# TrevorS/voxtral-mini-realtime-rs

Hardware: AMD Instinct MI355X
Metric: decode_tok_per_s (higher is better)
Workload: dtype f32

## Files before the change

voxtral-mini-realtime-rs_amd/csrc/vox_api.cpp:

```cpp
#include "vox_page_pool.h"
#include "vox_dev_base.h"
#include "vox_snapshot.h"
#include "vox_kv_bf16.h"

#include <algorithm>
#include <array>
#include <cassert>
#include <cmath>
#include <cstdio>
#include <cstdlib>
#include <cstring>
#include <deque>
#include <map>
#include <string>
#include <thread>
#include <vector>

using namespace vox;
using namespace vox_host;

namespace vox_host {
void binding_release(EngBinding& b) {
    for (void* p : {(void*)b.tab, (void*)b.part_val, (void*)b.part_idx}) if (p) (void)hipFree(p);
    if (b.err_word) (void)hipHostFree(b.err_word);
// ... 374 lines not shown
        if (f.w2 == PF::W2_F32) return q4_linear_dev(cx, L->w2.w, nullptr, ffn, F, M, x, D, EPI_RESID, x, D);
        if (f.w2 == PF::W2_PLANES_ROWS) HIPCHK(launch_xf_rows(ffn, F, M, F, cx->xf_scratch, s));
        return planes_from_xf(L->w2.w, f.kz_w2);
    };
    for (int l = 0; l < c.dec_layers; l++) {
        L = &m->dec[l]; kl = kc->k + (size_t)l * kc->layer_stride; vl = kc->v + (size_t)l * kc->layer_stride;
        VOXCHK(forms[l].f32_rows() ? layer_f32() : layer_xf(forms[l], l ? forms[l - 1].kz_w2 : 0));
    }
    if (!forms.empty() && forms.back().kz_w2) HIPCHK(launch_splitk_finish_resid(cx->kz_scratch, forms.back().kz_w2, M, D, x, D, s));
    return VOX_OK;
}

static bool decode_layer_fuses_attn_wo(const vox_model* m, const DecLayer& L, const AttnParams& ap, const vox_cache* kc) {
    const vox_model_cfg& c = m->cfg; const int D = c.dec_dim;
    return attn_wo_supported(ap, L.wo.w, c.dec_head_dim, kc->max_seq) && L.w13.w.fmt == WFMT_Q4_0 && L.w2.w.fmt == WFMT_Q4_0  && L.wo.w.N == D && D % 4 == 0 && L.w13.w.K == 3072 &&
           q4_gemv_default_R(L.w13.w.N, L.w13.w.K, EPI_SWIGLU) == 2;
}

static int32_t wo_acc_clear(vox_model* m, hipStream_t s) { if (m->d_wo_acc) HIPCHK(hipMemsetAsync(m->d_wo_acc, 0, (size_t)m->cfg.dec_layers * m->cfg.dec_dim * 8, s)); return VOX_OK; }
struct DecRingStep { const float* rope; int mask; };
static int32_t decoder_step_dev(vox_model* m, float* h, vox_cache* kc, const int* pos_ptr, int pos_off, const DecRingStep* ring = nullptr) {
    const vox_model_cfg& c = m->cfg; hipStream_t s = m->ctx->stream;
    const int D = c.dec_dim, H = c.dec_heads, KV = c.dec_kv_heads, hd = c.dec_head_dim, QD = H * hd, KD = KV * hd, F = c.dec_ffn;
    const size_t lf = kc->layer_stride;
    for (int l = 0; l < c.dec_layers; l++) {
        const DecLayer& L = m->dec[l]; float* kl = kc->k + (size_t)l * lf; float* vl = kc->v + (size_t)l * lf;
        GemvParams p{};
        p.w = L.wqkv.w; p.x = h; p.x_stride = D; p.out = m->d_q; p.out_stride = QD; p.gamma = L.attn_norm; p.eps = c.norm_eps;
        p.pos_ptr = pos_ptr; p.pos_off = pos_off; p.rope_cos = m->dec_cos; p.rope_sin = m->dec_sin; p.hd = hd; p.n_q = QD; p.n_k = KD;
        p.kcache = kl; p.vcache = vl; p.cache_head_stride = kc->max_seq * hd;
        if (ring) { p.rope_cos = ring->rope; p.rope_sin = ring->rope + hd / 2; p.rope_mask = ring->mask; }
        {
            HIPCHK(launch_q4_gemv(p, 1, PRO_RMS, ring ? EPI_ROPE_KV_RING : EPI_ROPE_KV, q4_gemv_default_R(p.w.N, p.w.K, EPI_ROPE_KV), s));
            AttnParams ap{}; ap.q = m->d_q; ap.k = kl; ap.v = vl; ap.kv_row_stride = hd; ap.kv_head_stride = kc->max_seq * hd; ap.out = m->d_att;
            ap.n_heads = H; ap.n_kv_heads = KV; ap.offset = pos_off; ap.window = c.dec_window; ap.pos_ptr = pos_ptr; ap.M = 1; ap.spec_rows = kc->max_seq;
            const int R13 = q4_gemv_default_R(L.w13.w.N, L.w13.w.K, EPI_SWIGLU);
            if (!ring && decode_layer_fuses_attn_wo(m, L, ap, kc) && h != m->d_h2) {
                long long* acc = m->d_wo_acc + (size_t)l * D;
                HIPCHK(launch_attn_wo(ap, L.wo.w, acc, kc->max_seq, s));
                GemvParams f{}; f.w = L.w13.w; f.x = h; f.x_stride = D; f.out = m->d_act; f.out_stride = F; f.gamma = L.ffn_norm; f.mul = L.ada_mul; f.eps = c.norm_eps;
                f.xacc = acc; f.x_out = m->d_h2;
                HIPCHK(launch_q4_gemv(f, 1, PRO_RMS_MUL_SUM, EPI_SWIGLU, R13, s));
                GemvParams d{}; d.w = L.w2.w; d.x = m->d_act; d.x_stride = F; d.out = h; d.out_stride = D; d.resid = m->d_h2; d.resid_stride = D;
                d.zero_acc = acc; d.zero_n = D;
                HIPCHK(launch_q4_gemv(d, 1, PRO_NONE, EPI_RESID, q4_gemv_default_R(d.w.N, d.w.K, EPI_RESID), s));
                continue;
            }
            HIPCHK(ring ? launch_attn_decode_ring(ap, hd, kc->max_seq, s) : launch_attn_decode(ap, hd, kc->max_seq, s));
        }
        GemvParams o{}; o.w = L.wo.w; o.x = m->d_att; o.x_stride = QD; o.out = h; o.out_stride = D; o.resid = h; o.resid_stride = D;
        HIPCHK(launch_q4_gemv(o, 1, PRO_NONE, EPI_RESID, q4_gemv_default_R(o.w.N, o.w.K, EPI_RESID), s));
        GemvParams f{}; f.w = L.w13.w; f.x = h; f.x_stride = D; f.out = m->d_act; f.out_stride = F; f.gamma = L.ffn_norm; f.mul = L.ada_mul; f.eps = c.norm_eps;
        HIPCHK(launch_q4_gemv(f, 1, PRO_RMS_MUL, EPI_SWIGLU, q4_gemv_default_R(f.w.N, f.w.K, EPI_SWIGLU), s));
        GemvParams d{}; d.w = L.w2.w; d.x = m->d_act; d.x_stride = F; d.out = h; d.out_stride = D; d.resid = h; d.resid_stride = D;
        HIPCHK(launch_q4_gemv(d, 1, PRO_NONE, EPI_RESID, q4_gemv_default_R(d.w.N, d.w.K, EPI_RESID), s));
    }
    return VOX_OK;
}

static int32_t engine_stream_prepare(vox_model* m) {
    const vox_model_cfg& c = m->cfg; hipStream_t s = m->ctx->stream;
    if (m->eng_ready || !m->eng_ok) return VOX_OK;
    const size_t sb = eng_stream_bytes(c.dec_layers, c.vocab);
    if (!m->eng_stream) {
        hipError_t e = hipMalloc((void**)&m->eng_stream, sb);
        if (e == hipSuccess) e = hipMalloc((void**)&m->eng_state, eng_state_bytes());
        if (e != hipSuccess) {
            (void)hipGetLastError();
            if (m->eng_stream) (void)hipFree(m->eng_stream); if (m->eng_state) (void)hipFree(m->eng_state);
            m->eng_stream = nullptr; m->eng_state = nullptr; m->eng_ok = false; m->eng_on = false; m->engb_ok = false;
            fprintf(stderr, "[voxtral_hip] decode engine: allocating the %.2f GB weight stream failed (%s); the launch-based decode paths are used\n", sb / 1e9, hipGetErrorString(e));
            return VOX_OK;
        }
    }
    HIPCHK(hipMemsetAsync(m->eng_stream, 0, sb, s)); HIPCHK(hipMemsetAsync(m->eng_state, 0, eng_state_bytes(), s));
    for (int l = 0; l < c.dec_layers; l++) {
        const DecLayer& L = m->dec[l];
        HIPCHK(launch_eng_pack(L.wqkv.w, 0, l, c.dec_layers, m->eng_stream, c.vocab, s)); HIPCHK(launch_eng_pack(L.wo.w, 1, l, c.dec_layers, m->eng_stream, c.vocab, s));
        HIPCHK(launch_eng_pack(L.w13.w, 2, l, c.dec_layers, m->eng_stream, c.vocab, s)); HIPCHK(launch_eng_pack(L.w2.w, 3, l, c.dec_layers, m->eng_stream, c.vocab, s));
    }
    HIPCHK(launch_eng_pack(m->tok.w, 4, 0, c.dec_layers, m->eng_stream, c.vocab, s));
    m->eng_ready = true;
    return VOX_OK;
}
static bool engb_prepare(vox_model* m, int n_grp) {
    if (!m->engb_ok || !m->engb_on || n_grp > 4) return false;
    if (engine_stream_prepare(m) != VOX_OK || !m->eng_ready) return false;
    if (engb_prepare_kernels() != hipSuccess) { (void)hipGetLastError(); m->engb_ok = false; return false; }
    if (!m->eng_wob) {
        const vox_model_cfg& c = m->cfg; hipStream_t s = m->ctx->stream;
        hipError_t e = hipMalloc((void**)&m->eng_wob, engb_wo_stream_bytes(c.dec_layers));
        if (e == hipSuccess) e = hipMemsetAsync(m->eng_wob, 0, engb_wo_stream_bytes(c.dec_layers), s);
        for (int l = 0; l < c.dec_layers && e == hipSuccess; l++) e = launch_eng_pack(m->dec[l].wo.w, 5, l, c.dec_layers, m->eng_wob, c.vocab, s);
        if (e != hipSuccess) { (void)hipGetLastError(); if (m->eng_wob) { (void)hipFree(m->eng_wob); m->eng_wob = nullptr; } m->engb_ok = false; return false; }
    }
    for (int gi = 0; gi < n_grp; gi++) {
        if (m->engb_state[gi]) continue;
        hipError_t e = hipMalloc((void**)&m->engb_state[gi], engb_state_bytes());
        if (e == hipSuccess) e = hipMalloc((void**)&m->engb_tab[gi], sizeof(EngLayerTab) * 32);
        if (e == hipSuccess) e = engb_state_init(m->engb_state[gi], m->ctx->stream);
        if (e != hipSuccess) { (void)hipGetLastError(); if (m->engb_state[gi]) { (void)hipFree(m->engb_state[gi]); m->engb_state[gi] = nullptr; } return false; }
    }
    return true;
}
static int32_t engine_strike(vox_model* m) {
    m->eng_strikes++;
    HIPCHK(hipMemsetAsync(m->eng_state, 0, eng_state_bytes(), m->ctx->stream)); m->eng_launches = 0; graphs_destroy(m);
    if (m->eng_strikes >= 3) { m->eng_ok = false; m->eng_on = false; }
    return VOX_OK;
}
static const int ENGINE_MAX_ROWS = 1024;
static void dec_layer_tab(const vox_model* m, float* k, float* v, size_t layer_stride, size_t group_off, EngLayerTab* out) {
    for (size_t l = 0, o = group_off; l < (size_t)m->cfg.dec_layers; l++, o += layer_stride) out[l] = EngLayerTab{m->dec[l].attn_norm, m->dec[l].ffn_norm, m->dec[l].ada_mul, k + o, v + o};
}
static bool engine_serves(const vox_model* m, const vox_cache* kc) { return m->eng_ok && m->eng_on && !m->eng_suspended && kc && kc->max_seq <= ENGINE_MAX_ROWS; }
static hipError_t engine_tab_enqueue(vox_model* m, EngBinding& b, const vox_cache* kc) {
    b.host.resize(m->cfg.dec_layers); dec_layer_tab(m, kc->k, kc->v, kc->layer_stride, 0, b.host.data());
    const hipError_t e = hipMemcpyAsync(b.tab, b.host.data(), sizeof(EngLayerTab) * b.host.size(), hipMemcpyHostToDevice, m->ctx->stream);
    b.cache = e == hipSuccess ? kc : nullptr; b.gen = kc->gen; return e;
}
static hipError_t binding_alloc(const vox_model* m, EngBinding& b, uint64_t* bytes = nullptr) {
    hipError_t e = hipSuccess; auto A = [&](void** q, size_t n) { if (e == hipSuccess && !*q && (e = hipMalloc(q, n)) == hipSuccess && bytes) *bytes += n; };
    A((void**)&b.tab, sizeof(EngLayerTab) * std::max(m->cfg.dec_layers, 32)); A((void**)&b.part_val, 256 * 4); A((void**)&b.part_idx, 256 * 4);
    if (e == hipSuccess && !b.err_word) { e = hipHostMalloc((void**)&b.err_word, 8, hipHostMallocDefault); if (e == hipSuccess) b.err_word[0] = b.err_word[1] = 0u; else b.err_word = nullptr; }
    return e;
}
static bool engine_bind(vox_model* m, EngBinding& b, const vox_cache* kc) {
    if (!engine_serves(m, kc) || engine_stream_prepare(m) != VOX_OK || !m->eng_ready) return false;
    hipError_t e = binding_alloc(m, b);
    if (e == hipSuccess && (b.cache != kc || b.gen != kc->gen)) { e = engine_tab_enqueue(m, b, kc); if (e == hipSuccess) e = hipStreamSynchronize(m->ctx->stream); }
    if (e != hipSuccess) { (void)hipGetLastError(); b.cache = nullptr; }
    return e == hipSuccess;
}
static EngParams engine_params(vox_model* m, const EngBinding& b, const vox_cache* kc, const float* h_in, const int* pos_ptr, int pos_off, float* logits_out) {
    const vox_model_cfg& c = m->cfg;
    EngParams ep{}; ep.stream = m->eng_stream; ep.cu_stride = eng_stream_bytes(c.dec_layers, c.vocab) / 256; ep.layers = b.tab; ep.n_layers = c.dec_layers; ep.h_in = h_in; ep.final_norm = m->dec_norm;
    ep.pos_ptr = pos_ptr; ep.pos_off = pos_off; ep.rope_cos = m->dec_cos; ep.rope_sin = m->dec_sin; ep.max_seq = kc->max_seq; ep.window = c.dec_window; ep.eps = c.norm_eps;
    eng_state_carve(m->eng_state, &ep); ep.part_val = b.part_val; ep.part_idx = b.part_idx; ep.logits_out = logits_out; ep.vocab = c.vocab; ep.tl = nullptr; ep.tl_layer = -1;
    ep.flags = m->eng_flags; ep.pace_ticks = (m->eng_flags & 512) ? 0 : m->eng_pace; ep.ag_delay_ticks = (m->eng_flags & 512) ? m->eng_pace : 0;
    return ep;
}
static int32_t engine_take_serials(vox_model* m, unsigned long long n, hipStream_t s) {
    if (m->eng_launches + n > (1ull << 25)) { HIPCHK(hipMemsetAsync(m->eng_state, 0, eng_state_bytes(), s)); m->eng_launches = 0; }
    m->eng_launches += n; return VOX_OK;
}
static int32_t engine_err_enqueue(vox_model* m, unsigned* dst, hipStream_t s) {
    EngParams ep{}; eng_state_carve(m->eng_state, &ep); HIPCHK(hipMemcpyAsync(dst, ep.err, 8, hipMemcpyDeviceToHost, s)); return VOX_OK;
}
static std::string engine_timeout_text(unsigned e, int strikes) {
    char b[96]; const int n = snprintf(b, sizeof b, "hand-off timeout (code %u, workgroup %u)", e & 0xff, (e >> 8) & 0xff);
    if (strikes > 0) snprintf(b + n, sizeof b - n, ", strike %d of 3", strikes);
    return b;
}
struct EngSuspend { vox_model* m; bool was; explicit EngSuspend(vox_model* m_) : m(m_), was(m_->eng_suspended) { m->eng_suspended = true; } ~EngSuspend() { m->eng_suspended = was; } };

extern "C" int32_t vox_model_set_decode_engine(vox_model* m, int32_t on, int32_t* active) {
    ARGCHK(m, "null argument"); VOXCHK(ctx_bind(m->ctx));
    const bool want = on != 0 && m->eng_ok;
    if (want != m->eng_on) { HIPCHK(hipStreamSynchronize(m->ctx->stream)); graphs_destroy(m); m->eng_on = want; }
    if (active) *active = m->eng_on ? 1 : 0;
    return VOX_OK;
}

extern "C" int32_t vox_model_set_batch_engine(vox_model* m, int32_t on, int32_t* active, uint64_t* launches) {
    ARGCHK(m, "null argument");
    if (on >= 0) m->engb_on = on != 0;
    if (active) *active = m->engb_ok && m->engb_on ? 1 : 0;
    if (launches) *launches = m->engb_launches;
    return VOX_OK;
}

static int32_t lm_head_argmax_dev(vox_model* m, const float* h, float* logits_out) {
    const vox_model_cfg& c = m->cfg;
    ARGCHK(c.dec_dim <= 4096, "lm_head GEMV is instantiated for dec_dim <= 4096 (got %d)", c.dec_dim);
    GemvParams p{}; p.w = m->tok.w; p.x = h; p.x_stride = c.dec_dim; p.out = logits_out; p.out_stride = c.vocab; p.gamma = m->dec_norm; p.eps = c.norm_eps;
    p.part_val = m->d_part_val; p.part_idx = m->d_part_idx;
    if (m->tok.w.fmt == WFMT_Q4_0) m->n_parts = q4_gemv_grid_k(c.vocab, c.dec_dim, m->argmax_R, EPI_ARGMAX);
    HIPCHK(launch_q4_gemv(p, 1, PRO_RMS, EPI_ARGMAX, m->argmax_R, m->ctx->stream));
    return VOX_OK;
}

static int32_t ensure_decode_state(vox_model* m, int S) {
    if (!m->cache || m->cache->max_seq < S) {
        int cap = std::max(S, 256); cap = std::min((cap + 255) / 256 * 256, m->dec_rope_len);
        ARGCHK(S <= cap, "sequence of %d decoder positions exceeds the RoPE table (%d)", S, m->dec_rope_len);
        if (m->cache) { HIPCHK(hipStreamSynchronize(m->ctx->stream)); cache_release(m->cache); m->eng_offline.cache = nullptr; }
        graphs_destroy(m);
        VOXCHK(cache_alloc(m, cap, &m->cache));
    }
    if (!m->d_tokens) { m->tokens_cap = m->dec_rope_len + 2; HIPCHK(hipMalloc((void**)&m->d_tokens, (size_t)m->tokens_cap * 4)); }
    ARGCHK(S + 2 <= m->tokens_cap, "sequence of %d decoder positions exceeds the token buffer", S);
    return VOX_OK;
}

namespace vox_host {
void prefix_release(vox_model* m) {
    PrefixState& p = m->pfx;
    for (float** q : {&p.enc_kv, &p.audio, &p.dec_k, &p.dec_v}) { if (*q) (void)hipFree(*q); *q = nullptr; }
    p.enc_built = p.dec_built = false; p.enc_bytes = p.dec_bytes = 0; p.t_embed.clear();
}
}
static void prefix_bounds(const vox_model* m, int* RC, int* PC) {
    const vox_model_cfg& c = m->cfg; *RC = 0; *PC = 0;
    vox_pad_cfg pc; vox_pad_cfg_voxtral(&pc);
    const long left = (long)pad_left(&pc), R = c.reshape_factor;
    if (left < 200 || R < 1 || c.n_mels != 128 || (c.enc_head_dim != 64 && c.enc_head_dim != 128) || m->enc.empty() || m->dec.empty()) return;
    const long Fc = (left - 200) / 160, rows = Fc >= 3 ? (Fc - 3) / 4 + 1 : 0;
    const long pcn = VOX_PREFIX_TOKENS - 1;
    if (rows / R < pcn || pcn * R + 4 > m->enc_rope_len) return;
    *PC = (int)pcn; *RC = (int)(pcn * R);
}
static bool prefix_active(const vox_model* m) { int rc, pc; prefix_bounds(m, &rc, &pc); return m->pfx.on && rc > 0; }
static hipError_t prefix_tokens_enqueue(int* d_tokens, hipStream_t s) { return hipMemcpyAsync(d_tokens, PREFIX_TOKENS.t, sizeof PREFIX_TOKENS.t, hipMemcpyHostToDevice, s); }
static int32_t prefill_prefix_rows(vox_model* m, const float* audio, int rows) {
    const vox_model_cfg& c = m->cfg;
    if (!m->d_prefix) HIPCHK(hipMalloc((void**)&m->d_prefix, (size_t)VOX_PREFIX_TOKENS * c.dec_dim * 4));
    HIPCHK(launch_embed(m->tok.w, m->d_tokens, rows, audio, c.dec_dim, nullptr, 0, 0, m->d_prefix, m->ctx->stream));
    m->cache->len = 0;
    return decoder_prefill_dev(m, m->d_prefix, rows, m->cache, 0);
}
static int32_t prefix_build(vox_model* m, const float* t_embed) {
    PrefixState& p = m->pfx; const vox_model_cfg& c = m->cfg; vox_ctx* cx = m->ctx; hipStream_t s = cx->stream;
    int RC, PC; prefix_bounds(m, &RC, &PC);
    if (!p.on || RC <= 0) return VOX_OK;
    if (p.enc_built && p.dec_built && p.t_embed.size() == (size_t)c.dec_dim && !std::memcmp(p.t_embed.data(), t_embed, (size_t)c.dec_dim * 4)) return VOX_OK;
    const int QD = c.enc_heads * c.enc_head_dim, hd = c.dec_head_dim, KV = c.dec_kv_heads;
    p.RC = RC; p.PC = PC;
    const size_t rows_bytes = (size_t)PC * hd * 4, n_rows = (size_t)c.dec_layers * KV;
    {
        hipError_t e = hipSuccess;
        auto A = [&](float** q, size_t n) { if (e == hipSuccess && !*q) e = hipMalloc((void**)q, n); };
        A(&p.enc_kv, (size_t)c.enc_layers * RC * 2 * QD * 4); A(&p.audio, (size_t)PC * c.dec_dim * 4); A(&p.dec_k, rows_bytes * n_rows); A(&p.dec_v, rows_bytes * n_rows);
        if (e != hipSuccess) {
            (void)hipGetLastError(); prefix_release(m); p.on = false;
            fprintf(stderr, "[voxtral_hip] prefix state: allocating %.1f MB failed (%s); every call runs the full computation\n",
                    ((double)c.enc_layers * RC * 2 * QD * 4 + 2.0 * rows_bytes * n_rows) / 1e6, hipGetErrorString(e));
            return VOX_OK;
        }
    }
    if (!p.enc_built) {
        const int Tb = 4 * (RC + 4);
        p.enc_bytes = (uint64_t)c.enc_layers * RC * 2 * QD * 4 + (uint64_t)PC * c.dec_dim * 4;
        MelTables t; VOXCHK(ctx_mel_tables(cx, &t));
        DevBuf mel; HIPCHK(mel.alloc((size_t)c.n_mels * Tb * 4));
        HIPCHK(launch_mel(nullptr, 0, (long)Tb * 160, 0, nullptr, t, mel.as<float>(), Tb, 1, s));
        int S4 = 0; p.capture = p.enc_kv; p.capture_rows = RC;
        const int32_t r = encode_dev(m, mel.as<float>(), Tb, &S4);
        p.capture = nullptr; p.capture_rows = 0;
        VOXCHK(r); ARGCHK(S4 >= PC, "internal: prefix build gave %d audio rows", S4);
        HIPCHK(hipMemcpyAsync(p.audio, m->d_audio, (size_t)PC * c.dec_dim * 4, hipMemcpyDeviceToDevice, s));
        HIPCHK(hipStreamSynchronize(s));
        p.enc_built = true;
    }
    VOXCHK(vox_model_set_t_embed(m, t_embed));
    VOXCHK(ensure_decode_state(m, VOX_PREFIX_TOKENS));
    p.dec_bytes = 2 * (uint64_t)rows_bytes * n_rows;
    HIPCHK(prefix_tokens_enqueue(m->d_tokens, s));
    VOXCHK(prefill_prefix_rows(m, p.audio, PC));
    const size_t pitch = (size_t)m->cache->max_seq * hd * 4;
    ARGCHK(m->cache->layer_stride == (size_t)KV * m->cache->max_seq * hd, "internal: cache layout");
    HIPCHK(hipMemcpy2DAsync(p.dec_k, rows_bytes, m->cache->k, pitch, rows_bytes, n_rows, hipMemcpyDeviceToDevice, s));
    HIPCHK(hipMemcpy2DAsync(p.dec_v, rows_bytes, m->cache->v, pitch, rows_bytes, n_rows, hipMemcpyDeviceToDevice, s));
    HIPCHK(hipStreamSynchronize(s));
    p.t_embed.assign(t_embed, t_embed + c.dec_dim); p.dec_built = true;
    return VOX_OK;
}
static int32_t prefix_rows_into(vox_model* m, vox_cache* kc, hipStream_t s) {
    const vox_model_cfg& c = m->cfg; const PrefixState& P = m->pfx;
    const size_t rows_bytes = (size_t)P.PC * c.dec_head_dim * 4, n_rows = (size_t)c.dec_layers * c.dec_kv_heads, pitch = (size_t)kc->max_seq * c.dec_head_dim * 4;
    const size_t plane = (size_t)c.dec_kv_heads * kc->max_seq * c.dec_head_dim, src_layer = (size_t)c.dec_kv_heads * P.PC * c.dec_head_dim;
    if (kc->layer_stride == plane) {
        HIPCHK(hipMemcpy2DAsync(kc->k, pitch, P.dec_k, rows_bytes, rows_bytes, n_rows, hipMemcpyDeviceToDevice, s));
        HIPCHK(hipMemcpy2DAsync(kc->v, pitch, P.dec_v, rows_bytes, rows_bytes, n_rows, hipMemcpyDeviceToDevice, s));
    } else for (int l = 0; l < c.dec_layers; l++) {
        HIPCHK(hipMemcpy2DAsync(kc->k + (size_t)l * kc->layer_stride, pitch, P.dec_k + (size_t)l * src_layer, rows_bytes, rows_bytes, c.dec_kv_heads, hipMemcpyDeviceToDevice, s));
        HIPCHK(hipMemcpy2DAsync(kc->v + (size_t)l * kc->layer_stride, pitch, P.dec_v + (size_t)l * src_layer, rows_bytes, rows_bytes, c.dec_kv_heads, hipMemcpyDeviceToDevice, s));
    }
    kc->len = P.PC; return VOX_OK;
}
static bool prefix_usable(const vox_model* m, int T) {
    const PrefixState& p = m->pfx; const vox_model_cfg& c = m->cfg;
    if (!p.on || !p.enc_built || !p.dec_built || p.RC <= 0 || knob_str("VOX_ATTN_F32")) return false;
    const int S = enc_rows(T);
    return S / c.reshape_factor > VOX_PREFIX_TOKENS && S <= m->enc_rope_len;
}
extern "C" int32_t vox_model_set_prefix_cache(vox_model* m, int32_t on, int32_t* active) {
    ARGCHK(m, "null argument"); VOXCHK(ctx_bind(m->ctx));
    if (on >= 0) {
        m->pfx.on = on != 0;
        if (!m->pfx.on) { HIPCHK(hipStreamSynchronize(m->ctx->stream)); prefix_release(m); }
        else if (m->t_embed_set) { std::vector<float> te = m->t_embed_host; VOXCHK(prefix_build(m, te.data())); }
    }
    if (active) *active = prefix_active(m) ? 1 : 0;
    return VOX_OK;
}
extern "C" int32_t vox_model_prefix_info(const vox_model* m, int32_t out[4]) {
    ARGCHK(m && out, "null argument");
    int rc, pc; prefix_bounds(m, &rc, &pc);
    const uint64_t b = (m->pfx.enc_kv ? m->pfx.enc_bytes : 0) + (m->pfx.dec_k ? m->pfx.dec_bytes : 0);
    out[0] = m->pfx.enc_built && m->pfx.dec_built ? 1 : 0; out[1] = rc; out[2] = pc; out[3] = (int32_t)std::min<uint64_t>(b, 0x7fffffff);
    return VOX_OK;
}

static int32_t decode_step_enqueue(vox_model* m, float* logits_out, bool eng, StepLaunch how = StepLaunch::StepAndArgmax) {
    const vox_model_cfg& c = m->cfg; hipStream_t s = m->ctx->stream;
    if (eng) {
        EngParams ep = engine_params(m, m->eng_offline, m->cache, m->d_h, m->d_pos, 0, logits_out);
        if (how == StepLaunch::EngineArgmaxFirst) {
            ep.flags |= 65536; ep.h_in = nullptr; ep.tokens = m->d_tokens; ep.pos_rw = m->d_pos; ep.tok_qs = m->tok.w.qs; ep.tok_sc = m->tok.w.sc; ep.tok_nb = m->tok.w.nb; ep.audio = m->d_audio;
        }
        HIPCHK(launch_decode_engine(ep, s));
        if (how == StepLaunch::StepAndArgmax) HIPCHK(launch_argmax_embed(m->d_part_val, m->d_part_idx, 256, m->d_tokens, m->d_pos, m->tok.w, m->d_audio, c.dec_dim, m->d_h, s));
        return VOX_OK;
    }
    VOXCHK(decoder_step_dev(m, m->d_h, m->cache, m->d_pos, 0));
    VOXCHK(lm_head_argmax_dev(m, m->d_h, logits_out));
    HIPCHK(launch_argmax_embed(m->d_part_val, m->d_part_idx, m->n_parts, m->d_tokens, m->d_pos, m->tok.w, m->d_audio, c.dec_dim, m->d_h, s));
    return VOX_OK;
}

struct ClipPlan { int S = 0, n_ids = 0, first_pos = 0, steps = 0; bool on_prefix = false, want_logits = false; };
static ClipPlan plan_clip(int S, bool on_prefix, int PC, bool want_logits) {
    ClipPlan p; p.S = S; p.on_prefix = on_prefix; p.want_logits = want_logits;
    if (S < VOX_PREFIX_TOKENS) return p;
    p.n_ids = std::max(S - VOX_PREFIX_TOKENS, 1);
    p.first_pos = on_prefix ? PC : VOX_PREFIX_TOKENS;
    p.steps = on_prefix ? S - PC - 1 : std::max(S - VOX_PREFIX_TOKENS - 1, 0);
    return p;
}

static int32_t seed_clip(vox_model* m, const ClipPlan& plan, DevBuf& dlog, RoctxStage& stage) {
    const vox_model_cfg& c = m->cfg; hipStream_t s = m->ctx->stream;
    HIPCHK(prefix_tokens_enqueue(m->d_tokens, s));
    m->cache->len = 0;
    stage.begin("prefill");
    if (plan.on_prefix) {
        VOXCHK(prefix_rows_into(m, m->cache, s));
    } else {
        VOXCHK(prefill_prefix_rows(m, m->d_audio, plan.first_pos));
        m->cache->len = plan.first_pos;
        if (plan.want_logits) HIPCHK(dlog.alloc((size_t)plan.n_ids * c.vocab * 4));
        VOXCHK(lm_head_argmax_dev(m, m->d_prefix + (size_t)(plan.first_pos - 1) * c.dec_dim, dlog.as<float>()));
    }
    HIPCHK(hipMemcpyAsync(m->d_pos, &plan.first_pos, 4, hipMemcpyHostToDevice, s));
    if (!plan.on_prefix) HIPCHK(launch_argmax_final(m->d_part_val, m->d_part_idx, m->n_parts, m->d_tokens, m->d_pos, 0, 0, s));
    return VOX_OK;
}

namespace vox_host {
void graphs_destroy(vox_model* m) {
    DecodeGraphs& g = m->graphs;
    for (int i = 0; i < 2; i++) {
        if (g.exec[i]) { (void)hipGraphExecDestroy(g.exec[i]); g.exec[i] = nullptr; }
        if (g.graph[i]) { (void)hipGraphDestroy(g.graph[i]); g.graph[i] = nullptr; }
    }
}
}
static DecodeGraphs& graphs_for(vox_model* m, const DecodeGraphs::Key& key) {
    const DecodeGraphs::Key& k = m->graphs.key;
    if (k.cache != key.cache || k.audio != key.audio || k.unroll != key.unroll || k.launch != key.launch) { graphs_destroy(m); m->graphs.key = key; }
    return m->graphs;
}
static int32_t graph_capture(vox_model* m, int which, int n_steps, bool eng) {
    DecodeGraphs& g = m->graphs; hipStream_t s = m->ctx->stream;
    HIPCHK(hipStreamBeginCapture(s, hipStreamCaptureModeThreadLocal));
    int32_t r = VOX_OK;
    for (int i = 0; i < n_steps && r == VOX_OK; i++) r = decode_step_enqueue(m, nullptr, eng, g.key.launch);
    hipError_t ce = hipStreamEndCapture(s, &g.graph[which]);
    if (r != VOX_OK) return r;
    HIPCHK(ce);
    HIPCHK(hipGraphInstantiate(&g.exec[which], g.graph[which], nullptr, nullptr, 0));
    return VOX_OK;
}
static int decode_unroll(bool eng) { const char* e = knob_str("VOX_DECODE_UNROLL"); return e && atoi(e) >= 1 && atoi(e) <= 32 ? atoi(e) : eng ? 8 : 1; }
static int32_t replay_rest(vox_model* m, bool eng, int done, int steps) {
    DecodeGraphs& g = m->graphs; hipStream_t s = m->ctx->stream; const int U = g.key.unroll;
    if (U > 1 && !g.exec[1] && steps - done >= 2 * U) VOXCHK(graph_capture(m, 1, U, eng));
    while (U > 1 && g.exec[1] && steps - done >= U) { HIPCHK(hipGraphLaunch(g.exec[1], s)); done += U; m->timings.graph_replays += U; }
    while (done < steps) { HIPCHK(hipGraphLaunch(g.exec[0], s)); done++; m->timings.graph_replays++; }
    return VOX_OK;
}
static int32_t steps_eager_logits(vox_model* m, const ClipPlan& plan, bool eng, float* d_logits_all) {
    int32_t r = VOX_OK; for (int i = 0; i < plan.steps && r == VOX_OK; i++) r = decode_step_enqueue(m, d_logits_all + (size_t)(i + 1) * m->cfg.vocab, eng);
    return r;
}
static int32_t steps_replayed(vox_model* m, const ClipPlan& plan, bool eng) {
    const DecodeGraphs& g = graphs_for(m, {m->cache, m->d_audio, decode_unroll(eng), StepLaunch::StepAndArgmax});
    int done = 0;
    if (!g.exec[0]) {
        VOXCHK(decode_step_enqueue(m, nullptr, eng)); done = 1;
        HIPCHK(hipStreamSynchronize(m->ctx->stream));
        VOXCHK(graph_capture(m, 0, 1, eng));
    }
    return replay_rest(m, eng, done, plan.steps);
}
static int32_t steps_chained(vox_model* m, const ClipPlan& plan) {
    hipStream_t s = m->ctx->stream;
    const DecodeGraphs& g = graphs_for(m, {m->cache, m->d_audio, decode_unroll(true), StepLaunch::EngineArgmaxFirst});
    VOXCHK(decode_step_enqueue(m, nullptr, true, StepLaunch::EngineAlone));
    if (!g.exec[0]) { HIPCHK(hipStreamSynchronize(s)); VOXCHK(graph_capture(m, 0, 1, true)); }
    VOXCHK(replay_rest(m, true, 1, plan.steps));
    HIPCHK(launch_argmax_final(m->d_part_val, m->d_part_idx, 256, m->d_tokens, m->d_pos, 1, 1, s));
    return VOX_OK;
}
static int32_t run_decode_steps(vox_model* m, const ClipPlan& plan, bool eng, float* d_logits_all) {
    const vox_model_cfg& c = m->cfg; hipStream_t s = m->ctx->stream;
    if (plan.steps <= 0) return VOX_OK;
    VOXCHK(wo_acc_clear(m, s));
    HIPCHK(launch_embed(m->tok.w, m->d_tokens, 1, m->d_audio, c.dec_dim, m->d_pos, 0, 0, m->d_h, s));
    if (plan.want_logits) return steps_eager_logits(m, plan, eng, d_logits_all);
    const char* k = knob_str("VOX_ENGINE_ARGMAX_IN");
    return eng && !(k && k[0] == '0') ? steps_chained(m, plan) : steps_replayed(m, plan, eng);
}

struct ClipRecords { vox_token_score* scores; vox_token_alts* alts; int k; };
static int32_t clip_attempt(vox_model* m, const ClipPlan& plan, int32_t* out_ids, float* logits_host, const ClipRecords* rec, bool* eng_timed_out) {
    const vox_model_cfg& c = m->cfg; hipStream_t s = m->ctx->stream;
    *eng_timed_out = false;
    VOXCHK(ensure_decode_state(m, plan.S));
    const bool eng = engine_bind(m, m->eng_offline, m->cache); if (eng) VOXCHK(engine_take_serials(m, (unsigned long long)plan.S + 8, s));
    DevBuf dlog; RoctxStage stage;
    VOXCHK(seed_clip(m, plan, dlog, stage));
    float* const d_logits_all = dlog.as<float>();
    stage.begin("decode");
    VOXCHK(run_decode_steps(m, plan, eng, d_logits_all));
    HIPCHK(hipMemcpyAsync(out_ids, m->d_tokens + VOX_PREFIX_TOKENS, (size_t)plan.n_ids * 4, hipMemcpyDeviceToHost, s));
    if (logits_host) HIPCHK(hipMemcpyAsync(logits_host, d_logits_all, (size_t)plan.n_ids * c.vocab * 4, hipMemcpyDeviceToHost, s));
    DevBuf dsc, dal;
    if (rec) {
        if (rec->scores) HIPCHK(dsc.alloc((size_t)plan.n_ids * sizeof(TokenScore)));
        if (rec->alts) HIPCHK(dal.alloc((size_t)plan.n_ids * sizeof(TokenAlts)));
        HIPCHK(launch_records_rows(d_logits_all, plan.n_ids, c.vocab, rec->k, dsc.as<TokenScore>(), dal.as<TokenAlts>(), s));
        if (rec->scores) HIPCHK(hipMemcpyAsync(rec->scores, dsc.p, (size_t)plan.n_ids * sizeof(TokenScore), hipMemcpyDeviceToHost, s));
        if (rec->alts) HIPCHK(hipMemcpyAsync(rec->alts, dal.p, (size_t)plan.n_ids * sizeof(TokenAlts), hipMemcpyDeviceToHost, s));
    }
    const bool eng_used = eng && plan.steps > 0;
    if (eng_used) VOXCHK(engine_err_enqueue(m, m->eng_offline.err_word, s));
    HIPCHK(hipStreamSynchronize(s));
    stage.end();
    *eng_timed_out = eng_used && m->eng_offline.err_word[0] != 0;
    return VOX_OK;
}

static int32_t transcribe_dev(vox_model* m, const float* d_mel, int T, const float* t_embed, int32_t* out_ids, int32_t cap, int32_t* n_ids,
                              float* logits_host, bool from_padded_samples = false, const ClipRecords* rec = nullptr) {
    VOXCHK(vox_model_set_t_embed(m, t_embed));
    const bool pfx = from_padded_samples && !logits_host && !rec && prefix_usable(m, T);
    double t0 = now_ms();
    RoctxScope whole("transcribe_streaming");
    int S = 0; RoctxStage stage; stage.begin("encode_audio");
    VOXCHK(encode_dev(m, d_mel, T, &S, pfx ? m->pfx.RC : 0));
    HIPCHK(hipStreamSynchronize(m->ctx->stream));
    stage.end();
    m->timings.encode_ms = now_ms() - t0; t0 = now_ms();
    *n_ids = 0; m->timings.decode_tokens = 0; m->timings.graph_replays = 0;
    const ClipPlan plan = plan_clip(S, pfx, m->pfx.PC, logits_host != nullptr || rec != nullptr);
    if (plan.n_ids == 0) { m->timings.decode_ms = 0; return VOX_OK; }
    ARGCHK(cap >= plan.n_ids, "out_ids capacity %d < %d", cap, plan.n_ids);
    bool timed_out = false;
    VOXCHK(clip_attempt(m, plan, out_ids, logits_host, rec, &timed_out));
    if (timed_out) {
        const unsigned e = m->eng_offline.err_word[0];
        VOXCHK(engine_strike(m));
        fprintf(stderr, "[voxtral_hip] decode engine: %s; this utterance is decoded again on the per-operator path%s\n",
                engine_timeout_text(e, m->eng_strikes).c_str(), m->eng_strikes >= 3 ? ", the engine is switched off" : "");
        int32_t r; { EngSuspend off(m); r = clip_attempt(m, plan, out_ids, logits_host, rec, &timed_out); }
        graphs_destroy(m);
        if (r != VOX_OK) return r;
    }
    m->cache->len = plan.first_pos + plan.steps;
    *n_ids = plan.n_ids; m->timings.decode_tokens = plan.n_ids;
    m->timings.decode_ms = now_ms() - t0;
    return VOX_OK;
}

extern "C" int32_t vox_encode_audio(vox_model* m, const float* mel, int32_t T, float* out, int32_t cap_rows, int32_t* S, int32_t mem_kind) {
    ARGCHK(m && mel && out && S, "null argument"); ARGCHK(T > 0, "empty mel"); VOXCHK(ctx_bind(m->ctx));
    const vox_model_cfg& c = m->cfg; hipStream_t s = m->ctx->stream;
    const float* d_mel = mel;
    if (mem_kind == VOX_MEM_HOST) {
        VOXCHK(ensure(&m->d_mel, &m->mel_cap, (size_t)c.n_mels * T));
        HIPCHK(hipMemcpyAsync(m->d_mel, mel, (size_t)c.n_mels * T * 4, hipMemcpyHostToDevice, s)); d_mel = m->d_mel;
    }
    int S4 = 0; VOXCHK(encode_dev(m, d_mel, T, &S4));
    ARGCHK(cap_rows >= S4, "output capacity %d rows < %d", cap_rows, S4);
    if (S4 > 0) HIPCHK(hipMemcpyAsync(out, m->d_audio, (size_t)S4 * c.dec_dim * 4, mem_kind == VOX_MEM_HOST ? hipMemcpyDeviceToHost : hipMemcpyDeviceToDevice, s));
    HIPCHK(hipStreamSynchronize(s));
    *S = S4; return VOX_OK;
}

extern "C" int32_t vox_transcribe_streaming(vox_model* m, const float* mel, int32_t T, const float* t_embed, int32_t* out_ids, int32_t cap,
                                            int32_t* n_ids, float* logits, int32_t mem_kind) {
    ARGCHK(m && mel && t_embed && out_ids && n_ids, "null argument"); ARGCHK(T > 0, "empty mel"); VOXCHK(ctx_bind(m->ctx));
    const vox_model_cfg& c = m->cfg; hipStream_t s = m->ctx->stream;
    const float* d_mel = mel;
    m->timings = vox_timings{};
    if (mem_kind == VOX_MEM_HOST) {
        VOXCHK(ensure(&m->d_mel, &m->mel_cap, (size_t)c.n_mels * T));
        HIPCHK(hipMemcpyAsync(m->d_mel, mel, (size_t)c.n_mels * T * 4, hipMemcpyHostToDevice, s)); d_mel = m->d_mel;
    }
    VOXCHK(transcribe_dev(m, d_mel, T, t_embed, out_ids, cap, n_ids, logits));
    m->timings.total_ms = m->timings.preprocess_ms + m->timings.encode_ms + m->timings.decode_ms;
    return VOX_OK;
}

static int32_t clip_front_end(vox_model* m, const float* samples, size_t n, int32_t mem_kind, int* T_out) {
    vox_ctx* cx = m->ctx; hipStream_t s = cx->stream;
    const float* d_s = samples;
    if (mem_kind == VOX_MEM_HOST) {
        VOXCHK(ensure(&m->d_samples, &m->samples_cap, n));
        HIPCHK(hipMemcpyAsync(m->d_samples, samples, n * 4, hipMemcpyHostToDevice, s)); d_s = m->d_samples;
    }
    vox_pad_cfg pc; vox_pad_cfg_voxtral(&pc);
    const size_t left = pad_left(&pc), right = pad_right(&pc, n + left), total = left + n + right, T = total / 160;
    MelTables t; VOXCHK(ctx_mel_tables(cx, &t));
    VOXCHK(ensure(&m->d_mel, &m->mel_cap, (size_t)128 * T));
    HIPCHK(launch_absmax(d_s, (long)n, 0.95f, cx->d_scale, s));
    HIPCHK(launch_mel(d_s, (long)n, (long)left, (long)right, cx->d_scale, t, m->d_mel, (int)T, 1, s));
    *T_out = (int)T;
    return VOX_OK;
}
static int32_t records_args_check(const void* scores, const void* alts, int32_t k) {
    ARGCHK(k >= 0 && k <= VOX_MAX_ALTERNATIVES, "k %d out of range (0..%d)", k, VOX_MAX_ALTERNATIVES);
    ARGCHK(k > 0 || !alts, "alts given with k == 0: k in 1..%d asks for alternatives", VOX_MAX_ALTERNATIVES);
    ARGCHK(k == 0 || alts, "k %d needs the alts array", k);
    ARGCHK(scores || alts, "scores and alts are both null: the unscored call serves that");
    return VOX_OK;
}
static int32_t transcribe_audio_impl(vox_model* m, const float* samples, size_t n, const float* t_embed, int32_t* out_ids, int32_t cap,
                                     int32_t* n_ids, int32_t mem_kind, const ClipRecords* rec);
extern "C" int32_t vox_transcribe_audio(vox_model* m, const float* samples, size_t n, const float* t_embed, int32_t* out_ids, int32_t cap,
                                        int32_t* n_ids, int32_t mem_kind) {
    return transcribe_audio_impl(m, samples, n, t_embed, out_ids, cap, n_ids, mem_kind, nullptr);
}
extern "C" int32_t vox_transcribe_audio_scored(vox_model* m, const float* samples, size_t n, const float* t_embed, int32_t* out_ids, int32_t cap, int32_t* n_ids,
                                               vox_token_score* scores, vox_token_alts* alts, int32_t k, int32_t mem_kind) {
    ARGCHK(m, "null model"); ARGCHK(samples && t_embed && out_ids, "null argument"); ARGCHK(n_ids, "null n_ids"); ARGCHK(n > 0, "empty audio");
    VOXCHK(records_args_check(scores, alts, k));
    ARGCHK(mem_kind == VOX_MEM_HOST || mem_kind == VOX_MEM_DEVICE, "bad mem_kind %d", mem_kind);
    const ClipRecords rec{scores, alts, k};
    return transcribe_audio_impl(m, samples, n, t_embed, out_ids, cap, n_ids, mem_kind, &rec);
}
static int32_t transcribe_audio_impl(vox_model* m, const float* samples, size_t n, const float* t_embed, int32_t* out_ids, int32_t cap,
                                     int32_t* n_ids, int32_t mem_kind, const ClipRecords* rec) {
    ARGCHK(m && samples && t_embed && out_ids && n_ids, "null argument"); ARGCHK(n > 0, "empty audio"); VOXCHK(ctx_bind(m->ctx));
    const vox_model_cfg& c = m->cfg; hipStream_t s = m->ctx->stream;
    ARGCHK(c.n_mels == 128, "the log-mel front-end produces 128 bins; model expects %d", c.n_mels);
    m->timings = vox_timings{};
    VOXCHK(prefix_build(m, t_embed));
    const double t0 = now_ms();
    int T = 0; VOXCHK(clip_front_end(m, samples, n, mem_kind, &T));
    HIPCHK(hipStreamSynchronize(s));
    m->timings.preprocess_ms = now_ms() - t0;
    VOXCHK(transcribe_dev(m, m->d_mel, T, t_embed, out_ids, cap, n_ids, nullptr, true, rec));
    m->timings.total_ms = m->timings.preprocess_ms + m->timings.encode_ms + m->timings.decode_ms;
    return VOX_OK;
}

static const int32_t VOX_RETRY_ON_LAUNCHES = -1000;
template <class Run> static int32_t retry_on_launches(Run run) { int32_t r = run(true); if (r == VOX_RETRY_ON_LAUNCHES) r = run(false); return r; }
struct BatchDrain { vox_ctx* c; ~BatchDrain() { (void)hipStreamSynchronize(c->stream); if (c->fe_stream) (void)hipStreamSynchronize(c->fe_stream); } };
static int32_t batch_lengths(const vox_model* m, int n, const float* const* samples, const size_t* n_samples, const int32_t* caps, const int* slot_of,
                             std::vector<int>& T, std::vector<int>& S, std::vector<int>& len, int* Smax) {
    const int PREFIX_LEN = VOX_PREFIX_TOKENS;
    vox_pad_cfg pc; vox_pad_cfg_voxtral(&pc);
    T.assign(n, 0); S.assign(n, 0); len.assign(n, 0); *Smax = 0;
    for (int i = 0; i < n; i++) {
        ARGCHK(samples[i] && n_samples[i] > 0, "empty audio in batch slot %d", slot_of[i]);
        const size_t left = pad_left(&pc), total = left + n_samples[i] + pad_right(&pc, n_samples[i] + left);
        T[i] = (int)(total / 160); S[i] = conv_len(conv_len(T[i])) / m->cfg.reshape_factor; *Smax = std::max(*Smax, S[i]);
        const int cnt_i = S[i] >= PREFIX_LEN ? std::max(S[i] - PREFIX_LEN, 1) : 0;
        ARGCHK(caps[i] >= cnt_i, "out_ids[%d] capacity %d < %d", slot_of[i], caps[i], cnt_i);
        len[i] = S[i] >= PREFIX_LEN ? std::max(S[i], PREFIX_LEN + 1) : 0;
    }
    ARGCHK(*Smax <= m->dec_rope_len, "sequence too long for the decoder RoPE table");
    return VOX_OK;
}
static int32_t front_end_units(const MelTables& mt, int i0, int nu, const float* const* samples, const size_t* n_samples, const int* T, const float* const* unit_scale,
                               float* smp, float* mel, float* scale, const float** d_mels, hipStream_t sf) {
    vox_pad_cfg pc; vox_pad_cfg_voxtral(&pc);
    size_t mo = 0, so = 0;
    for (int k = 0; k < nu; k++) {
        const int i = i0 + k; const float* d_s = samples[i];
        if (smp) { float* dst = smp + so; so += n_samples[i]; HIPCHK(hipMemcpyAsync(dst, samples[i], n_samples[i] * 4, hipMemcpyHostToDevice, sf)); d_s = dst; }
        const size_t left = pad_left(&pc), right = pad_right(&pc, n_samples[i] + left);
        float* mel_i = mel + mo; mo += (size_t)128 * T[i]; d_mels[k] = mel_i;
        if (!unit_scale) HIPCHK(launch_absmax(d_s, (long)n_samples[i], 0.95f, scale + k, sf));
        HIPCHK(launch_mel(d_s, (long)n_samples[i], (long)left, (long)right, unit_scale ? unit_scale[i] : scale + k, mt, mel_i, T[i], 1, sf));
    }
    return VOX_OK;
}
static int32_t upload_prefix(int n, int tstride, const std::vector<int>& len, int* d_tok, int* d_pos, int* d_len, hipStream_t s) {
    std::vector<int32_t> prefix((size_t)n * tstride, 0); std::vector<int> pos0(n, VOX_PREFIX_TOKENS - 1);
    for (int i = 0; i < n; i++) std::copy(PREFIX_TOKENS.t, PREFIX_TOKENS.t + VOX_PREFIX_TOKENS, prefix.begin() + (size_t)i * tstride);
    HIPCHK(hipMemcpyAsync(d_tok, prefix.data(), prefix.size() * 4, hipMemcpyHostToDevice, s)); HIPCHK(hipMemcpyAsync(d_pos, pos0.data(), (size_t)n * 4, hipMemcpyHostToDevice, s));
    HIPCHK(hipMemcpyAsync(d_len, len.data(), (size_t)n * 4, hipMemcpyHostToDevice, s));
    HIPCHK(hipStreamSynchronize(s));
    return VOX_OK;
}
static int32_t copy_out_ids(int n, const std::vector<int>& S, int tstride, const int* d_tok, int32_t* const* out_ids, int32_t* n_ids, int* total, hipStream_t s) {
    const int PREFIX_LEN = VOX_PREFIX_TOKENS;
    std::vector<int32_t> host_tok((size_t)n * tstride);
    HIPCHK(hipMemcpyAsync(host_tok.data(), d_tok, host_tok.size() * 4, hipMemcpyDeviceToHost, s));
    HIPCHK(hipStreamSynchronize(s)); *total = 0;
    for (int i = 0; i < n; i++) {
        const int cnt = S[i] >= PREFIX_LEN ? std::max(S[i] - PREFIX_LEN, 1) : 0;
        if (cnt > 0) std::memcpy(out_ids[i], host_tok.data() + (size_t)i * tstride + PREFIX_LEN, (size_t)cnt * 4);
        n_ids[i] = cnt; *total += cnt;
    }
    return VOX_OK;
}
static int32_t engb_timeout_check(vox_model* m, int n_blk, bool continuous, hipStream_t s) {
    for (int b = 0; b < n_blk; b++) { EngBParams ep{}; engb_state_carve(m->engb_state[b], &ep); HIPCHK(hipMemcpyAsync(m->engb_err_host[b], ep.err, 8, hipMemcpyDeviceToHost, s)); }
    HIPCHK(hipStreamSynchronize(s));
    for (int b = 0; b < n_blk; b++) if (m->engb_err_host[b][0]) {
        const unsigned e = m->engb_err_host[b][0];
        m->engb_strikes++;
        char grp[32] = ""; if (!continuous) snprintf(grp, sizeof grp, ", group %d", b);
        fprintf(stderr, "[voxtral_hip] batched decode engine%s: hand-off timeout (code %u, workgroup %u%s), strike %d of 3; re-running the %s on the launch-based step%s\n",
                continuous ? " (continuous batch)" : "", e & 0xff, (e >> 8) & 0xff, grp, m->engb_strikes, continuous ? "session" : "batch", m->engb_strikes >= 3 ? ", the engine is switched off" : "");
        for (int gj = 0; gj < 4; gj++) if (m->engb_state[gj]) (void)engb_state_init(m->engb_state[gj], s);
        if (m->engb_strikes >= 3) m->engb_ok = false;
        return VOX_RETRY_ON_LAUNCHES;
    }
    return VOX_OK;
}
struct StepGraphs {
    hipStream_t s; std::vector<std::pair<uint32_t, hipGraphExec_t>> ex; std::vector<hipGraph_t> gr;
    explicit StepGraphs(hipStream_t st) : s(st) {} StepGraphs(const StepGraphs&) = delete; StepGraphs& operator=(const StepGraphs&) = delete;
    ~StepGraphs() { (void)hipStreamSynchronize(s); for (auto& e : ex) if (e.second) (void)hipGraphExecDestroy(e.second); for (auto g : gr) if (g) (void)hipGraphDestroy(g); }
    hipGraphExec_t find(uint32_t a) const { for (auto& e : ex) if (e.first == a) return e.second; return nullptr; }
    template <class Step> int32_t capture(uint32_t act, Step& step, hipGraphExec_t* out) {
        HIPCHK(hipStreamBeginCapture(s, hipStreamCaptureModeThreadLocal));
        const int32_t r = step(act);
        hipGraph_t graph = nullptr;
        const hipError_t ce = hipStreamEndCapture(s, &graph);
        if (graph) gr.push_back(graph);
        if (r != VOX_OK) return r;
        HIPCHK(ce);
        const hipError_t ie = hipGraphInstantiate(out, graph, nullptr, nullptr, 0);
        if (ie != hipSuccess) return fail(VOX_ERR_HIP, "hipGraphInstantiate: %s", hipGetErrorString(ie));
        ex.emplace_back(act, *out);
        return VOX_OK;
    }
};
static size_t xf_bytes(int K) { return (size_t)2 * (K / 128) * 256 * 16; }

extern "C" int32_t vox_debug_attn_gqa_max_seq(vox_ctx* c, int32_t* out) {
    ARGCHK(c && out, "null argument"); VOXCHK(ctx_bind(c));
    int most = 0; HIPCHK(attn_decode_gqa_max_seq(&most));
    *out = most; return VOX_OK;
}
static int32_t attn_decode_debug(vox_ctx* c, const vox_attn_decode_desc* d, const float* q, const void* k, const void* v, void* out, bool ring, int tab_len = 0, bool bf16 = false) {
    ARGCHK(c && d && q && k && v && out, "null argument"); ARGCHK(d->pos, "null argument (pos)");
    ARGCHK(d->head_dim == 128, "head_dim %d: the decoder's decode attention serves head_dim 128 alone", d->head_dim);
    ARGCHK(d->n_seq >= 1 && d->n_seq <= 4096, "n_seq %d out of range (1..4096)", d->n_seq);
    ARGCHK(d->n_heads >= 1 && d->n_kv_heads >= 1 && d->n_heads <= 64 && d->n_heads % d->n_kv_heads == 0, "bad head counts (%d query heads, %d KV heads)", d->n_heads, d->n_kv_heads);
    ARGCHK(d->window >= -1, "window %d (-1: none)", d->window);
    ARGCHK(d->n_slices >= 1 && d->n_slices <= 4096 && (d->kv_row || d->n_slices >= d->n_seq), "n_slices %d: without kv_row every sequence reads its own slice (n_seq %d)", d->n_slices, d->n_seq);
    for (int i = 0; d->kv_row && i < d->n_seq; i++) ARGCHK(d->kv_row[i] >= 0 && d->kv_row[i] < d->n_slices, "kv_row[%d] = %d outside the %d slices", i, d->kv_row[i], d->n_slices);
    const bool paged = d->page_rows != 0;
    const int hd = 128, H = d->n_heads, KV = d->n_kv_heads, QD = H * hd, W = QD + 2 * KV * hd, n = d->n_seq;
    int shift = 0;
    if (ring) {
        ARGCHK(d->max_seq >= 1 && d->max_seq <= 16384, "max_seq %d (the ring capacity) out of range (1..16384)", d->max_seq);
        ARGCHK(!paged && !d->pool_pages && !d->page_tab && !d->page_tab_stride && !d->score_rows, "a ring call takes no paged field");
        ARGCHK(!d->prefer_gqa && !d->spec && !d->out_xf, "the ring form is the per-head kernel writing f32 rows: prefer_gqa, spec and out_xf must be 0");
        ARGCHK(d->window >= 0 && d->window + 1 <= d->max_seq, "window %d: a ring of %d rows serves windows 0..%d", d->window, d->max_seq, d->max_seq - 1);
        for (int i = 0; i < n; i++) ARGCHK(d->pos[i] >= 0 && d->pos[i] < (1 << 24), "pos[%d] = %d outside 0..2^24 - 1", i, d->pos[i]);
    } else if (!paged) {
        ARGCHK(d->max_seq >= 1 && d->max_seq <= 16384, "max_seq %d out of range (1..16384)", d->max_seq);
        ARGCHK(!d->pool_pages && !d->page_tab && !d->page_tab_stride && !d->score_rows, "a slab call takes no paged field");
        for (int i = 0; i < n; i++) ARGCHK(d->pos[i] >= 0 && d->pos[i] < d->max_seq, "pos[%d] = %d outside the cache's %d rows", i, d->pos[i], d->max_seq);
    } else {
        ARGCHK(d->page_rows >= 16 && d->page_rows <= 1024 && !(d->page_rows & (d->page_rows - 1)), "page_rows %d is not a power of two in 16..1024", d->page_rows);
        while ((1 << shift) < d->page_rows) shift++;
        ARGCHK(d->page_tab, "null argument (page_tab)"); ARGCHK(!d->max_seq && !d->spec, "a paged call takes no max_seq and has no speculative form");
        ARGCHK(d->pool_pages >= 1 && d->pool_pages <= (1 << 20), "pool_pages %d out of range", d->pool_pages);
        ARGCHK(d->page_tab_stride >= 1 && d->page_tab_stride <= 1024, "page_tab_stride %d out of range (1..1024)", d->page_tab_stride);
        ARGCHK(d->score_rows >= 1 && d->score_rows <= 16384, "score_rows %d out of range (1..16384)", d->score_rows);
        if (tab_len) {
            ARGCHK(d->window >= 0, "a ring table needs a sliding window (window %d)", d->window);
            ARGCHK(tab_len <= d->page_tab_stride, "page_tab_len %d exceeds page_tab_stride %d", tab_len, d->page_tab_stride);
            ARGCHK(tab_len >= d->window / d->page_rows + 2 + 2, "page_tab_len %d: a window of %d in pages of %d rows needs a ring table of at least %d entries (the window's %d pages + 2)", tab_len,
                   d->window, d->page_rows, d->window / d->page_rows + 4, d->window / d->page_rows + 2);
        }
        for (int i = 0; i < n; i++) {
            const int pos = d->pos[i], row = d->kv_row ? d->kv_row[i] : i;
            if (tab_len) ARGCHK(pos >= 0 && pos < (1 << 24), "pos[%d] = %d outside 0..2^24 - 1", i, pos);
            else
            ARGCHK(pos >= 0 && (pos >> shift) < d->page_tab_stride, "pos[%d] = %d outside the table's %d pages of %d rows", i, pos, d->page_tab_stride, d->page_rows);
            const int j_lo = d->window >= 0 ? std::max(0, pos - d->window) : 0;
            ARGCHK(pos - j_lo + 1 <= d->score_rows, "pos[%d] = %d attends %d keys, score_rows is %d", i, pos, pos - j_lo + 1, d->score_rows);
            for (int pg = j_lo >> shift; pg <= (pos >> shift); pg++) {
                const int e = d->page_tab[(size_t)row * d->page_tab_stride + (tab_len ? pg % tab_len : pg)];
                ARGCHK(e >= 0 && e < d->pool_pages, "sequence %d: table entry %d of its window is %d, outside the pool's %d pages", i, pg, e, d->pool_pages);
            }
        }
    }
    VOXCHK(ctx_bind(c));
    if (!paged && d->prefer_gqa && attn_decode_takes_gqa(hd, H, KV)) {
        int most = 0; HIPCHK(attn_decode_gqa_max_seq(&most));
        ARGCHK(d->max_seq <= most, "max_seq %d: the slab GQA form serves at most %d rows per KV head", d->max_seq, most);
    }
    hipStream_t s = c->stream;
    const size_t slice_f = paged ? (size_t)KV * d->page_rows * hd : (size_t)KV * d->max_seq * hd, kv_f = slice_f * (paged ? d->pool_pages : d->n_slices);
    const int n_grp = (n + 15) / 16; const size_t xf_b = xf_bytes(QD);
    DevBuf dq, dk, dv, dout, dxf, dint;
    const size_t tab_n = paged ? (size_t)d->n_slices * d->page_tab_stride : 0;
    const size_t kv_b = kv_f * (bf16 ? 2 : 4);
    HIPCHK(dq.alloc((size_t)n * W * 4)); HIPCHK(dk.alloc(kv_b)); HIPCHK(dv.alloc(kv_b)); HIPCHK(dout.alloc((size_t)n * QD * 4)); HIPCHK(dxf.alloc(xf_b * n_grp));
    HIPCHK(dint.alloc((2 * (size_t)n + tab_n) * 4));
    int* d_pos = dint.as<int>(); int* d_row = d_pos + n; int* d_tab = d_row + n;
    HIPCHK(hipMemsetAsync(dq.p, 0, (size_t)n * W * 4, s));
    HIPCHK(hipMemcpy2DAsync(dq.p, (size_t)W * 4, q, (size_t)QD * 4, (size_t)QD * 4, n, hipMemcpyHostToDevice, s));
// ... 3141 lines not shown
```

voxtral-mini-realtime-rs_amd/csrc/vox_engine.hip:

```cpp
#include "vox_kernels.h"

#include <hip/hip_fp16.h>

#include <cstdio>
#include <cstdlib>

namespace vox {
namespace {

#include "vox_engine_common.h"

__global__ __launch_bounds__(64) void eng_pack_lm_kernel(Q4W w, unsigned char* __restrict__ stream, size_t op_off, int vocab) {
    const int q = blockIdx.x, b = blockIdx.y, lane = threadIdx.x;
    const int row = lm_rows_per_cu(vocab) * b + q;
    unsigned char* dst = stream + (size_t)NCU * (op_off + (size_t)(q / NCONS) * PK_A) + (size_t)b * PK_A + (size_t)(q % NCONS) * PASS_A;
    const size_t src = (size_t)row * w.nb + lane;
    reinterpret_cast<uint4*>(dst)[lane] = w.qs[src];
    reinterpret_cast<uint16_t*>(dst + PA_S0)[lane] = w.sc[src];
    const size_t sh = (size_t)row * w.nb + 64 + (lane >> 1);
    const uint4 qh = w.qs[sh];
    reinterpret_cast<uint2*>(dst + PA_Q1)[lane] = (lane & 1) ? make_uint2(qh.z, qh.w) : make_uint2(qh.x, qh.y);
    if ((lane & 1) == 0) reinterpret_cast<uint16_t*>(dst + PA_S1)[lane >> 1] = w.sc[sh];
}
__global__ __launch_bounds__(64) void eng_pack_kernel(Q4W w, int op, unsigned char* __restrict__ stream, size_t op_off) {
    const int pk = blockIdx.x / (NCONS * 4), wv = (blockIdx.x / 4) % NCONS, s = blockIdx.x % 4, b = blockIdx.y, lane = threadIdx.x, n = lane & 15, g = lane >> 4;
    const int steps = pk_steps(op, pk); const bool half = pk_half_tile(op, pk);
    if (s >= steps || (half && n >= 8)) return;
    int tile, T; rec_src(op, pk, wv, s, &tile, &T);
    const int row = tile_row(op, b, tile, n), blk0 = step_blk0(op, b, T);
    const size_t pk_bytes = (size_t)op_pk_bytes(op), rec_bytes = half ? REC_H : REC;
    unsigned char* dst = stream + (size_t)NCU * (op_off + (size_t)pk * pk_bytes) + (size_t)b * pk_bytes + (size_t)wv * steps * rec_bytes + (size_t)s * rec_bytes;
    const uint4 q = w.qs[(size_t)row * w.nb + blk0 + (g >> 1)];
    reinterpret_cast<uint2*>(dst)[half ? g * 8 + n : lane] = (g & 1) ? make_uint2(q.z, q.w) : make_uint2(q.x, q.y);
    if (g < 2) reinterpret_cast<uint16_t*>(dst + (half ? REC_H_SC : REC_SC))[(half ? 8 : 16) * g + n] = w.sc[(size_t)row * w.nb + blk0 + g];
}

struct EngCtl {
    unsigned ring_ready[8], ring_done[8];
    unsigned xs0_flag, xs1_flag, xa_flag, qkv_flag;
    unsigned cbar, dead, gathering, gw_flag;
    unsigned xcd_ok, xcc_id, ag_flag, pub_cnt;
    float rstd0, rstd1, pad1, pad2;
    float best_val[16]; int best_idx[16];
    float h_own[16], h1_own[16];
    unsigned ag_done, pad_q[3];
    float rope_c[24], rope_s[24];
};
constexpr int L_RING = 0;
constexpr int L_XS = L_RING + NSLOT * SLOT_BYTES;
constexpr int L_U = L_XS + ED * 4;
constexpr int L_XA = L_U;
constexpr int L_PART = L_U;
constexpr int L_SC = L_U;
constexpr int L_PO = L_SC + SC_MAX * 4;
constexpr int L_PL = L_PO + 12 * 128 * 4;
constexpr int L_QKVN = L_PL + 64;
constexpr int L_TMP = L_QKVN + 384 * 4;
constexpr int L_SSQ = L_TMP + 384 * 4;
constexpr int L_BLK = L_SSQ + NCU * 4;
constexpr int L_TAB = L_BLK + 96 * 8;
constexpr int MAX_LAYERS = 32;
constexpr int L_GW = L_TAB + MAX_LAYERS * (int)sizeof(EngLayerTab);
constexpr int L_CTL = L_GW + (MAX_LAYERS + 1) * 32 * 4;
constexpr int L_TOTAL = L_CTL + (int)sizeof(EngCtl);
static_assert(L_TOTAL <= 160 * 1024, "LDS budget");
static_assert(L_TAB % 16 == 0 && sizeof(EngLayerTab) == 40, "layer table");
static_assert(L_XS % 16 == 0 && L_XA % 16 == 0 && L_QKVN % 16 == 0 && L_PO % 16 == 0 && L_CTL % 16 == 0 && L_BLK % 8 == 0 && 72 * 12 * 4 <= SC_MAX * 4 && 1152 * 4 + 96 * 6 * 4 <= SC_MAX * 4 + 12 * 128 * 4, "aligned carve");

__device__ __forceinline__ void eng_loader(const EngParams& p, EngCtl* c, unsigned ring_lds, int lane, const Tl& tl) {
    Loader<EngCtl, NSLOT> ld; ld.c = c; ld.err = p.err; ld.ring_lds = ring_lds; ld.voff = (unsigned)lane * 16u; ld.thin = (p.flags & 1) != 0; ld.pace = (u64)p.pace_ticks;
    const bool fake = (p.flags & 2) != 0;
    const bool nodma = (p.flags & 32) != 0;
    if (p.flags & 64) ld.pause_ticks = 300;
    if (p.flags & 1024) ld.depth = 2;
    if (p.flags & 2048) ld.depth = 1;
    const u64 base = (u64)p.stream;
    const unsigned n_layer_pk = (unsigned)p.n_layers * PK_LAYER, n_pk = n_layer_pk + (unsigned)lm_packets(p.vocab);
    unsigned l = 0, r = 0;
    u64 off = 0;
#pragma unroll 1
    for (unsigned pk = 0; pk < n_pk; pk++) {
        int bytes = PK_A;
        if (pk < n_layer_pk) {
            if (r < PK_LAYER_M) bytes = PK_M;
            if (r == 0 && (int)l == p.tl_layer) tl(16);
        } else { ld.pace = 0; ld.pause_ticks = 0; ld.depth = 3; }
        const u64 src = fake ? base + (u64)blockIdx.x * PK_A : base + (u64)NCU * off + (u64)blockIdx.x * (u64)bytes;
        if (bytes == PK_M) ld.issue<PK_M>(src, lane, nodma); else ld.issue<PK_A>(src, lane, nodma);
        off += (u64)bytes;
        if (++r == PK_LAYER) { if ((int)l == p.tl_layer) tl(17); r = 0; l++; }
    }
    ld.flush();
    tl(18);
}


__device__ __forceinline__ void comm_probe_x(const EngParams& p, EngCtl* c, int lane, const u64* src, unsigned tag, const Tl& tl, bool T) {
    const srd_t sd = make_srd(src, ED * 8u);
    if (T) tl(20);
    u64 t0 = 0;
    if (p.flags & 512) {
        const u64 tw = wall_clock64();
        while (wall_clock64() - tw < (u64)p.ag_delay_ticks) __builtin_amdgcn_s_sleep(1);
    } else
    for (;;) {
        const u64 gq = ld_gran(sd, 48u * (unsigned)lane);
        if (__all((unsigned)(gq >> 32) == tag)) break;
        if (sweep_bail(t0, tag, c, p.err)) break;
    }
    if (T) tl(21);
}
__device__ __forceinline__ void comm_publish_rows(const EngParams& p, int lane, float hraw, float gw, u64* dst, u64* ssq, unsigned tag, float* own) {
    const int b = blockIdx.x;
    float sq = lane < OWN ? hraw * hraw : 0.f;
    sq = row16_sum_e(sq);
    if (lane < OWN) { publish(dst + OWN * b + lane, tag, hraw * gw); own[lane] = hraw; }
    if (lane == 0) publish(ssq + b, tag, sq);
}

constexpr int ENGF_ARGMAX_IN = 65536;
__device__ __forceinline__ float comm_next_input(const EngParams& p, int lane, unsigned own_k) {
    float xv[4]; int xi[4];
#pragma unroll
    for (int u = 0; u < 4; u++) { xv[u] = as_g(p.part_val)[lane + 64 * u]; xi[u] = ((const __attribute__((address_space(1))) int*)(uintptr_t)p.part_idx)[lane + 64 * u]; }
    const int cur = __builtin_amdgcn_readfirstlane(*p.pos_rw) + 1;
    const float au = as_g(p.audio)[(size_t)cur * ED + own_k];
    float bv = -INFINITY; int bi = 0x7fffffff;
#pragma unroll
    for (int u = 0; u < 4; u++) if (xv[u] > bv || (xv[u] == bv && xi[u] < bi)) { bv = xv[u]; bi = xi[u]; }
#define ENG_AMAX_STEP(CTRL) { const float ov = dppf<CTRL>(bv); const int oi = dppi<CTRL>(bi); if (ov > bv || (ov == bv && oi < bi)) { bv = ov; bi = oi; } }
    ENG_AMAX_STEP(0xB1) ENG_AMAX_STEP(0x4E) ENG_AMAX_STEP(0x141) ENG_AMAX_STEP(0x140)
#undef ENG_AMAX_STEP
    float v0 = rlf(bv, 0); int token = __builtin_amdgcn_readlane(bi, 0);
#pragma unroll
    for (int r = 1; r < 4; r++) { const float ov = rlf(bv, 16 * r); const int oi = __builtin_amdgcn_readlane(bi, 16 * r); if (ov > v0 || (ov == v0 && oi < token)) { v0 = ov; token = oi; } }
    if (blockIdx.x == 0 && lane == 0) p.tokens[cur] = token;
    token = (unsigned)token < (unsigned)p.vocab ? token : 0;
    const unsigned c = own_k >> 5, e = own_k & 31;
    const size_t blk = (size_t)token * (size_t)p.tok_nb + c;
    const unsigned byte = ((const __attribute__((address_space(1))) unsigned char*)(uintptr_t)p.tok_qs)[blk * 16 + (e & 15)];
    const float d = __half2float(__ushort_as_half(((const __attribute__((address_space(1))) unsigned short*)(uintptr_t)p.tok_sc)[blk]));
    const int nib = e < 16 ? (int)(byte & 15u) : (int)(byte >> 4);
    return __fadd_rn(au, __fmul_rn(__fsub_rn((float)nib, 8.0f), d));
}

__device__ __forceinline__ void eng_comm(const EngParams& p, EngCtl* c, unsigned char* lds, const int lane0, const Tl& tl) {
    const int b = blockIdx.x, g = b & 7, j = b >> 3, h = 4 * g + (j >> 3);
    float* xa = reinterpret_cast<float*>(lds + L_XA); float* qkvn = reinterpret_cast<float*>(lds + L_QKVN);
    float* tmp = reinterpret_cast<float*>(lds + L_TMP);
    const EngLayerTab* tab = reinterpret_cast<const EngLayerTab*>(lds + L_TAB);
    const unsigned tag_base = (*p.serial + 1u) * 64u;
    const bool PROBE_SMALL = (p.flags & 4) != 0;
    const int own_r = min(lane0, OWN - 1);
    const unsigned own_k = (unsigned)(OWN * b + own_r);
    const float* gwt = reinterpret_cast<const float*>(lds + L_GW);
    {
        const float g0 = ld_gf(make_srd(p.n_layers > 0 ? tab[0].attn_norm : p.final_norm, ED * 4u), own_k) * (p.n_layers > 0 ? 1.0f : 512.0f);
        const float hraw = (p.flags & ENGF_ARGMAX_IN) ? comm_next_input(p, lane0, own_k) : ld_gf(make_srd(p.h_in, ED * 4u), own_k);
        comm_publish_rows(p, lane0, hraw, g0, p.H0, p.SS0, tag_base, c->h_own);
    }
#pragma unroll 1
    for (int st = 0; st <= 2 * p.n_layers; st++) {
        int lane = lane0; asm volatile("" : "+v"(lane));
        const int l = st >> 1; const bool odd = st & 1, last = st == 2 * p.n_layers, T = l == p.tl_layer;
        const unsigned tag = tag_base + (unsigned)l + 1u;
        if (odd) comm_probe_x(p, c, lane, p.H1, tag, tl, T);
        else comm_probe_x(p, c, lane, p.H0, tag - 1u, tl, false);
        lds_st(&c->gathering, 1u);
        lds_st(&c->ag_flag, (unsigned)st + 1u);
        if (T) tl(odd ? 11 : 8);
        if (p.flags & (1 | 64)) wait_ge(&c->ag_done, NCONS * ((unsigned)st + 1u), c, p.err, ERR_STAGE);
        lds_st(&c->gathering, 0u);
        if (last) break;
        if (!odd) {
            wait_ge(&c->gw_flag, (unsigned)NCONS, c, p.err, ERR_STAGE);
            const bool xloc_nt = (p.flags & 128) != 0 && (p.flags & 4096) != 0 && lds_ld(&c->xcd_ok) != 0;
            {
                wait_ge(&c->pub_cnt, NCONS * (4u * (unsigned)l + 1u), c, p.err, ERR_STAGE);
                lds_st(&c->gathering, 1u);
                float v[6];
                sweep<6>(p.G, (EQD + 2 * EKD) * 8u, tag, [&](int u) { const int i = lane + 64 * u, seg = i >> 7, e = i & 127; return seg == 0 ? 128 * h + e : (seg == 1 ? EQD : EQD + EKD) + 128 * g + e; },
                         [&]() { return lane < 32 ? EQD + 128 * g + 4 * lane : EQD + EKD + 128 * g + 4 * (lane - 32); }, PROBE_SMALL, v, c, p.err, xloc_nt);
                lds_st(&c->gathering, 0u);
#pragma unroll
                for (int u = 0; u < 6; u++) qkvn[lane + 64 * u] = v[u];
                ENG_CFENCE(); lds_st(&c->qkv_flag, (unsigned)l + 1u);
            }
            if (T) tl(9);
            {
                wait_ge(&c->pub_cnt, NCONS * (4u * (unsigned)l + 2u), c, p.err, ERR_STAGE);
                lds_st(&c->gathering, 1u);
                float v[6];
                sweep<6>(p.PW, NPW * ED * 8u, tag, [&](int u) { const int i = lane + 64 * u, hh = i / OWN, r = i - hh * OWN; return hh * ED + OWN * b + r; }, [&]() { return (lane & 31) * ED + OWN * b; }, PROBE_SMALL, v, c, p.err);
#pragma unroll
                for (int u = 0; u < 6; u++) tmp[lane + 64 * u] = v[u];
                lds_st(&c->gathering, 0u);
                ENG_CFENCE();
                float a = 0.f;
                const int r = min(lane, OWN - 1);
#pragma unroll 4
                for (int hh = 0; hh < NPW; hh++) a += tmp[hh * OWN + r];
                wait_ge(&c->gw_flag, (unsigned)NCONS, c, p.err, ERR_STAGE);
                if (!((p.flags & 16384) && blockIdx.x == 7 && l == 1))
                    comm_publish_rows(p, lane, c->h_own[r] + a, gwt[(l * 2 + 1) * 16 + r], p.H1, p.SS1, tag, c->h1_own);
            }
            if (T) tl(10);
        } else {
            const bool xloc_nt = (p.flags & 128) != 0 && (p.flags & 4096) != 0 && lds_ld(&c->xcd_ok) != 0;
            {
                wait_ge(&c->pub_cnt, NCONS * (4u * (unsigned)l + 3u), c, p.err, ERR_STAGE);
                lds_st(&c->gathering, 1u);
                float v[18];
                sweep<18>(p.A, EF * 8u, tag, [&](int u) { return 1152 * g + lane + 64 * u; }, [&]() { return 1152 * g + 36 * (lane & 31) + 35; }, PROBE_SMALL, v, c, p.err, xloc_nt);
#pragma unroll
                for (int u = 0; u < 18; u++) xa[lane + 64 * u] = v[u];
                ENG_CFENCE(); lds_st(&c->xa_flag, (unsigned)l + 1u);
                lds_st(&c->gathering, 0u);
            }
            if (T) tl(12);
            {
                wait_ge(&c->pub_cnt, NCONS * (4u * (unsigned)l + 4u), c, p.err, ERR_STAGE);
                lds_st(&c->gathering, 1u);
                float v[2];
                sweep<2>(p.P2, NP2 * ED * 8u, tag, [&](int u) { const int i = min(lane + 64 * u, NP2 * OWN - 1), pp = i / OWN, r = i - pp * OWN; return pp * ED + OWN * b + r; }, [&]() { return min(lane, NP2 - 1) * ED + OWN * b; }, PROBE_SMALL, v, c, p.err);
#pragma unroll
                for (int u = 0; u < 2; u++) if (lane + 64 * u < NP2 * OWN) tmp[lane + 64 * u] = v[u];
                lds_st(&c->gathering, 0u);
                ENG_CFENCE();
                float a = 0.f;
                const int r = min(lane, OWN - 1);
#pragma unroll
                for (int pp = 0; pp < NP2; pp++) a += tmp[pp * OWN + r];
                comm_publish_rows(p, lane, c->h1_own[r] + a, gwt[((l + 1) * 2) * 16 + r], p.H0, p.SS0, tag, c->h_own);
            }
            if (T) tl(13);
        }
    }
}

__device__ __forceinline__ f2 cvt2(unsigned w, bool hi) { return hi ? __builtin_amdgcn_cvt_pk_f32_fp8((int)w, true) : __builtin_amdgcn_cvt_pk_f32_fp8((int)w, false); }
__device__ __forceinline__ float block_dot(const uint4 q, const f2* __restrict__ x, float init) {
    f2 a0 = {init, 0.f}, a1 = {0.f, 0.f};
    const unsigned w[4] = {q.x, q.y, q.z, q.w};
#pragma unroll
    for (int d = 0; d < 4; d++) {
        const unsigned lo = w[d] & 0x0F0F0F0Fu, hi = (w[d] >> 4) & 0x0F0F0F0Fu;
        a0 = __builtin_elementwise_fma(cvt2(lo, false), x[2 * d], a0);
        a1 = __builtin_elementwise_fma(cvt2(lo, true), x[2 * d + 1], a1);
        a0 = __builtin_elementwise_fma(cvt2(hi, false), x[8 + 2 * d], a0);
        a1 = __builtin_elementwise_fma(cvt2(hi, true), x[8 + 2 * d + 1], a1);
    }
    return (a0.x + a0.y) + (a1.x + a1.y);
}

__device__ __forceinline__ float half_dot(const uint2 q, const f2* __restrict__ x, float init) {
    f2 a0 = {init, 0.f}, a1 = {0.f, 0.f};
    const unsigned w[2] = {q.x, q.y};
#pragma unroll
    for (int d = 0; d < 2; d++) {
        const unsigned lo = w[d] & 0x0F0F0F0Fu, hi = (w[d] >> 4) & 0x0F0F0F0Fu;
        a0 = __builtin_elementwise_fma(cvt2(lo, false), x[4 * d], a0);
        a1 = __builtin_elementwise_fma(cvt2(lo, true), x[4 * d + 1], a1);
        a0 = __builtin_elementwise_fma(cvt2(hi, false), x[4 * d + 2], a0);
        a1 = __builtin_elementwise_fma(cvt2(hi, true), x[4 * d + 3], a1);
    }
    return (a0.x + a0.y) + (a1.x + a1.y);
}

struct XA {
    f2 x[16], xh[8]; float m8, m8h;
    __device__ __forceinline__ void load_chunk(const float* xs, int chunk) {
        asm volatile("" : "+v"(chunk));
        const float4* x4 = reinterpret_cast<const float4*>(xs);
        float s = 0.f;
#pragma unroll
        for (int jj = 0; jj < 8; jj++) {
            const float4 v = x4[sw_piece(chunk, jj)];
            x[2 * jj] = f2{v.x, v.y}; x[2 * jj + 1] = f2{v.z, v.w};
            s += (v.x + v.y) + (v.z + v.w);
        }
        m8 = s * (-1.0f / 64.0f);
    }
    __device__ __forceinline__ void load(const float* xs, int chunk, int chunk_h, int hb) {
        load_chunk(xs, chunk);
        asm volatile("" : "+v"(chunk_h));
        const float4* x4 = reinterpret_cast<const float4*>(xs);
        float s = 0.f;
#pragma unroll
        for (int d = 0; d < 2; d++)
#pragma unroll
            for (int hh = 0; hh < 2; hh++) {
                const float4 v = x4[sw_piece(chunk_h, 4 * hh + 2 * hb + d)];
                xh[4 * d + 2 * hh] = f2{v.x, v.y}; xh[4 * d + 2 * hh + 1] = f2{v.z, v.w};
                s += (v.x + v.y) + (v.z + v.w);
            }
        m8h = s * (-1.0f / 64.0f);
    }
};
struct PassA { uint4 q0; uint2 q1; float s0, s1; };

typedef int i4v __attribute__((ext_vector_type(4)));
struct StepCtx { i4v A; float m8sx, sxinv; };
__device__ __forceinline__ StepCtx load_ctx(const unsigned char* planes, const float2* binfo, int blk0, int lane) {
    const int n = lane & 15, g = lane >> 4;
    StepCtx cx; cx.A = i4v{0, 0, 0, 0};
    if (n < 8 && (g >> 1) == (n >> 2)) cx.A = *reinterpret_cast<const i4v*>(planes + (((blk0 + (n >> 2)) * 4 + (n & 3)) * 2 + (g & 1)) * 16);
    const float2 bi = binfo[blk0 + (g & 1)];
    cx.m8sx = bi.x; cx.sxinv = bi.y;
    return cx;
}
struct RecR { i4v B; float sc; };
__device__ __forceinline__ RecR rec_read(const unsigned char* rec, bool half, int lane) {
    const int n = lane & 15, g = lane >> 4;
    uint2 q = make_uint2(0u, 0u);
    if (!half) q = reinterpret_cast<const uint2*>(rec)[lane];
    else if (n < 8) q = reinterpret_cast<const uint2*>(rec)[g * 8 + n];
    const unsigned short sb = reinterpret_cast<const unsigned short*>(rec + (half ? REC_H_SC : REC_SC))[(half ? 8 : 16) * (g & 1) + (half ? (n & 7) : n)];
    RecR r;
    r.B[0] = (int)(q.x & 0x0F0F0F0Fu); r.B[1] = (int)(q.y & 0x0F0F0F0Fu); r.B[2] = (int)((q.x >> 4) & 0x0F0F0F0Fu); r.B[3] = (int)((q.y >> 4) & 0x0F0F0F0Fu);
    r.sc = __half2float(__ushort_as_half(sb));
    asm volatile("" : "+v"(r.B[0]), "+v"(r.B[1]), "+v"(r.B[2]), "+v"(r.B[3]), "+v"(r.sc));
    return r;
}
__device__ __forceinline__ float mstep(const RecR& r, const StepCtx& cx, float acc) {
    const i4v D = __builtin_amdgcn_mfma_i32_16x16x64_i8(cx.A, r.B, i4v{0, 0, 0, 0}, 0, 0, 0);
    const int lo = (int)((unsigned)D[0] + ((unsigned)D[1] << 7)), hi = (int)((unsigned)D[2] + ((unsigned)D[3] << 7));
    float t = fmaf((float)hi, 16384.0f, (float)lo);
    t += cx.m8sx;
    return fmaf(t, r.sc * cx.sxinv, acc);
}
__device__ __forceinline__ float mstep(const unsigned char* rec, bool half, int lane, const StepCtx& cx, float acc) { return mstep(rec_read(rec, half, lane), cx, acc); }
__device__ __forceinline__ float g01_sum(float v, int lane) { return v + __shfl(v, (lane + 16) & 63); }
__device__ __forceinline__ void to_digits(const float (&v)[4], int lane, unsigned char* plane_blk, float2* binfo_blk) {
    float mx = fmaxf(fmaxf(fabsf(v[0]), fabsf(v[1])), fmaxf(fabsf(v[2]), fabsf(v[3])));
    mx = fmaxf(mx, dppf<0xB1>(mx)); mx = fmaxf(mx, dppf<0x4E>(mx)); mx = fmaxf(mx, dppf<0x141>(mx));
    int e = __builtin_amdgcn_frexp_expf(mx);
    e = max(e, -100);
    const float f = ldexpf(1.0f, 26 - e);
    int xi[4];
#pragma unroll
    for (int i = 0; i < 4; i++) xi[i] = (int)rintf(v[i] * f);
    int s = (xi[0] + xi[1]) + (xi[2] + xi[3]);
    s += dppi<0xB1>(s); s += dppi<0x4E>(s); s += dppi<0x141>(s);
    if ((lane & 7) == 0) *binfo_blk = make_float2(-8.0f * (float)s, ldexpf(1.0f, e - 26));
    const int e0 = 4 * (lane & 7), h = (e0 >> 3) & 1, off = (e0 & 4) + 8 * (e0 >> 4);
#pragma unroll
    for (int cdig = 0; cdig < 4; cdig++) {
        unsigned d = 0;
#pragma unroll
        for (int i = 0; i < 4; i++) { const int dv = cdig < 3 ? (xi[i] >> (7 * cdig)) & 127 : xi[i] >> 21; d |= (unsigned)(dv & 0xFF) << (8 * i); }
        *reinterpret_cast<unsigned*>(plane_blk + (cdig * 2 + h) * 16 + off) = d;
    }
}

struct Cons {
    const EngParams& p; EngCtl* c; unsigned char* lds; int cw, lane; unsigned P; unsigned cbar_n;
    __device__ __forceinline__ Cons(const EngParams& p_, EngCtl* c_, unsigned char* lds_, int cw_, int lane_) : p(p_), c(c_), lds(lds_), cw(cw_), lane(lane_), P(0), cbar_n(0) {}
    __device__ __forceinline__ void cbarrier() {
        cbar_n += NCONS;
        ENG_CFENCE();
        if (lane == 0) __hip_atomic_fetch_add(&c->cbar, 1u, RLX, WG);
        wait_ge(&c->cbar, cbar_n, c, p.err, ERR_CBAR);
    }
    __device__ __forceinline__ void published(const Tl& tl, int evt) {
        ENG_CFENCE();
        if (lane == 0) { const unsigned old = __hip_atomic_fetch_add(&c->pub_cnt, 1u, RLX, WG); if (evt >= 0 && tl.buf && old % NCONS == NCONS - 1) tl.buf[evt] = wall_clock64(); }
    }
    __device__ __forceinline__ const unsigned char* slot_wait(unsigned pk, int share_bytes, int& slot) {
        slot = (int)(pk % NSLOT); const unsigned k = pk / NSLOT;
        wait_ge(&c->ring_ready[slot], k + 1u, c, p.err, ERR_RING);
        return lds + L_RING + slot * SLOT_BYTES + cw * share_bytes;
    }
    __device__ __forceinline__ void slot_release(int slot) {
        ENG_CFENCE();
        if (lane == 0) __hip_atomic_fetch_add(&c->ring_done[slot], 1u, RLX, WG);
    }
    __device__ __forceinline__ void fetch(unsigned pk, PassA& P_) {
        int slot; const unsigned char* base = slot_wait(pk, PASS_A, slot);
        P_.q0 = reinterpret_cast<const uint4*>(base)[lane];
        P_.q1 = reinterpret_cast<const uint2*>(base + PA_Q1)[lane];
        P_.s0 = __half2float(__ushort_as_half(reinterpret_cast<const unsigned short*>(base + PA_S0)[lane]));
        P_.s1 = __half2float(__ushort_as_half(reinterpret_cast<const unsigned short*>(base + PA_S1)[lane >> 1]));
        slot_release(slot);
    }
    static __device__ __forceinline__ float dot(const PassA& P_, const XA& xr) { return fmaf(P_.s1, half_dot(P_.q1, xr.xh, xr.m8h), P_.s0 * block_dot(P_.q0, xr.x, xr.m8)); }

    template <bool DIGITS>
    __device__ __forceinline__ float all_gather(const u64* src, const u64* ssq, unsigned tag, unsigned stage, unsigned char* xs, float* ssl, float2* binfo, const Tl& tl, bool T) {
        wait_ge(&c->ag_flag, stage + 1u, c, p.err, ERR_STAGE);
        const srd_t sd = make_srd(src, ED * 8u), qd = make_srd(ssq, NCU * 8u);
        int ln = lane; asm volatile("" : "+v"(ln));
        if (DIGITS) {
            const unsigned q = 64u * (unsigned)cw + (unsigned)ln;
            u32x4 ra, rb; u64 rq = 0, t0 = 0;
            for (;;) {
                ra = __builtin_bit_cast(u32x4, __builtin_amdgcn_raw_buffer_load_b128(sd, (int)(q * 32u), 0, 16));
                rb = __builtin_bit_cast(u32x4, __builtin_amdgcn_raw_buffer_load_b128(sd, (int)(q * 32u + 16u), 0, 16));
                if (cw < 4) rq = ld_gran(qd, 64u * (unsigned)cw + (unsigned)ln);
                bool ok = ra.y == tag && ra.w == tag && rb.y == tag && rb.w == tag;
                if (cw < 4) ok &= (unsigned)(rq >> 32) == tag;
                if (__all(ok)) break;
                if (sweep_bail(t0, tag, c, p.err)) break;
            }
            if (T) tl(22);
            if (ln == 0) __hip_atomic_fetch_add(&c->ag_done, 1u, RLX, WG);
            const float v[4] = {__uint_as_float(ra.x), __uint_as_float(ra.z), __uint_as_float(rb.x), __uint_as_float(rb.z)};
            to_digits(v, ln, xs + (q >> 3) * 128u, binfo + (q >> 3));
            if (cw < 4) ssl[64 * cw + ln] = __uint_as_float((unsigned)rq);
            return 0.f;
        }
        const unsigned q = 64u * (((unsigned)cw + blockIdx.x) % NCONS) + (unsigned)ln;
        u32x4 ra, rb; u64 rq = 0, t0 = 0;
        for (;;) {
            ra = __builtin_bit_cast(u32x4, __builtin_amdgcn_raw_buffer_load_b128(sd, (int)(q * 32u), 0, 16));
            rb = __builtin_bit_cast(u32x4, __builtin_amdgcn_raw_buffer_load_b128(sd, (int)(q * 32u + 16u), 0, 16));
            if (cw < 4) rq = ld_gran(qd, 64u * (unsigned)cw + (unsigned)ln);
            bool ok = ra.y == tag && ra.w == tag && rb.y == tag && rb.w == tag;
            if (cw < 4) ok &= (unsigned)(rq >> 32) == tag;
            if (__all(ok)) break;
            if (sweep_bail(t0, tag, c, p.err)) break;
        }
        if (ln == 0) __hip_atomic_fetch_add(&c->ag_done, 1u, RLX, WG);
        const float v[4] = {__uint_as_float(ra.x), __uint_as_float(ra.z), __uint_as_float(rb.x), __uint_as_float(rb.z)};
#pragma unroll
        for (int i = 0; i < 4; i++) reinterpret_cast<float*>(xs)[sw_dword((int)(4u * q) + i)] = v[i];
        if (cw < 4) ssl[64 * cw + ln] = __uint_as_float((unsigned)rq);
        cbarrier();
        return rstd_staged(ssl);
    }
    __device__ __forceinline__ float rstd_staged(const float* ssl) {
        const float ss = wave_sum_e((ssl[lane] + ssl[lane + 64]) + (ssl[lane + 128] + ssl[lane + 192]));
        return 1.0f / sqrtf(ss / (float)ED + p.eps);
    }
};

__device__ __forceinline__ void eng_consumer(const EngParams& p, EngCtl* c, unsigned char* lds, int cw, const int lane0, const Tl& tl) {
    Cons cs(p, c, lds, cw, lane0);
    const int b = blockIdx.x, g = b & 7, j = b >> 3, h = 4 * g + (j >> 3), s = j & 7;
    unsigned char* xs = lds + L_XS; float* ssl = reinterpret_cast<float*>(lds + L_SSQ);
    float2* binfo = reinterpret_cast<float2*>(lds + L_BLK);
    const float* xa = reinterpret_cast<const float*>(lds + L_XA);
    float* part = reinterpret_cast<float*>(lds + L_PART);
    float* part2 = reinterpret_cast<float*>(lds + L_XA + 1152 * 4);
    const float* qkvn = reinterpret_cast<const float*>(lds + L_QKVN);
    float* sc = reinterpret_cast<float*>(lds + L_SC); float2* po = reinterpret_cast<float2*>(lds + L_PO); float* pl = reinterpret_cast<float*>(lds + L_PL);
    const unsigned tag_base = (*p.serial + 1u) * 64u;
    const int pos = *p.pos_ptr + p.pos_off + ((p.flags & ENGF_ARGMAX_IN) ? 1 : 0);
    const int j_lo = p.window >= 0 ? max(0, pos - p.window) : 0, n_old = pos - j_lo, last_old = max(n_old - 1, 0);
    const int half = EHD / 2;
    if (cw == 0 && lane0 < 24) {
        float rc = 1.0f, rs = 0.0f;
        if (lane0 < 20) { const int pr = lane0 < 16 ? 8 * s + (lane0 >> 1) : 2 * j + ((lane0 - 16) >> 1); rc = p.rope_cos[(size_t)pos * half + pr]; rs = p.rope_sin[(size_t)pos * half + pr]; }
        c->rope_c[lane0] = rc; c->rope_s[lane0] = rs;
    }
    const float scale = 1.0f / sqrtf((float)EHD);
    const int n_items = 3 * p.n_layers, npass_lm = lm_passes(p.vocab), row0_lm = lm_rows_per_cu(p.vocab) * b;
    {
        const EngLayerTab* tab = reinterpret_cast<const EngLayerTab*>(lds + L_TAB);
        float* gwt = reinterpret_cast<float*>(lds + L_GW);
        const bool xchg = cw == NCONS - 1 && (p.flags & 128) != 0;
        const unsigned my = c->xcc_id;
        if (xchg && lane0 == 0) publish(p.XC + b, tag_base, __uint_as_float(my));
        const int l = cw + NCONS * (lane0 >> 4), r = lane0 & 15, lc = min(l, max(p.n_layers - 1, 0));
        const bool lok = r < OWN && l <= p.n_layers && (lane0 >> 4) < 3, lay = l < p.n_layers;
        const unsigned k = (unsigned)(OWN * b + min(r, OWN - 1));
        const gcf_p pa = as_g(lay ? tab[lc].attn_norm : p.final_norm);
        float wa = 0.f, wf = 0.f, wd = 0.f;
        if (lok) { wa = pa[k]; if (p.n_layers > 0) { wf = as_g(tab[lc].ffn_norm)[k]; wd = as_g(tab[lc].ada_mul)[k]; } }
        if (lok) {
            gwt[(l * 2) * 16 + r] = lay ? wa : wa * 512.0f;
            if (lay) gwt[(l * 2 + 1) * 16 + r] = wf * wd;
        }
        if (cw == NCONS - 1) {
            unsigned ok = 0;
            if (xchg) {
                float v[1];
                const bool got = sweep<1>(p.XC, NCU * 8u, tag_base, [&](int) { return 8 * (lane0 & 31) + g; }, [&]() { return 0; }, false, v, c, p.err);
                ok = got && __all(__float_as_uint(v[0]) == my) ? 1u : 0u;
                if (!ok && lane0 == 0) __hip_atomic_store(p.err + 1, 9u | ((unsigned)b << 8) | (my << 16), RLX, AG);
            }
            lds_st(&c->xcd_ok, ok);
        }
        ENG_CFENCE();
        if (lane0 == 0) __hip_atomic_fetch_add(&c->gw_flag, 1u, RLX, WG);
    }
    float best = -INFINITY; int best_i = 0x7fffffff;
    bool xloc = false;

#pragma unroll 1
    for (int it = 0; it <= n_items; it++) {
        int lane = lane0; asm volatile("" : "+v"(lane));
        const int l = it / 3, op = it == n_items ? (int)EOP_LM : (it - 3 * l == 0 ? (int)EOP_QKV : it - 3 * l == 1 ? (int)EOP_W13 : (int)EOP_W2);
        const bool T = l == p.tl_layer && cw == 0 && op != EOP_LM;
        const int tlev = l == p.tl_layer ? 1 : 0;
        const unsigned tag = tag_base + (unsigned)l + 1u;
        const EngLayerTab* L = reinterpret_cast<const EngLayerTab*>(lds + L_TAB) + (op == EOP_LM ? 0 : l);
        if (op == EOP_QKV) {
            const gf_p kc = as_g(L->kc) + (size_t)g * p.max_seq * EHD, vc = as_g(L->vc) + (size_t)g * p.max_seq * EHD;
            const int t12 = cw * 64 + lane;
            const int part_ = t12 & 7, ks = t12 >> 3;
            RecR rq[8];
            {
                int s0, s1, s2;
                const unsigned char* b0 = cs.slot_wait(cs.P, 2 * REC, s0);
                rq[0] = rec_read(b0, false, lane); rq[1] = rec_read(b0 + REC, false, lane);
                cs.slot_release(s0);
                const unsigned char* b1 = cs.slot_wait(cs.P + 1, 2 * REC, s1);
                rq[2] = rec_read(b1, false, lane); rq[3] = rec_read(b1 + REC, false, lane);
                cs.slot_release(s1);
                const unsigned char* b2 = cs.slot_wait(cs.P + 2, 4 * REC_H, s2);
#pragma unroll
                for (int i = 0; i < 4; i++) rq[4 + i] = rec_read(b2 + i * REC_H, true, lane);
                cs.slot_release(s2);
                cs.P += QKV_PK;
            }
            cs.all_gather<true>(p.H0, p.SS0, tag - 1u, 2u * (unsigned)l, xs, ssl, binfo, tl, false);
            if (T) tl(0);
            constexpr int NKP = 2;
            float4 kpre[NKP][4];
            auto kload = [&](int u) {
                const unsigned ko = (unsigned)(j_lo + min(ks + 96 * u, last_old)) * EHD + part_ * 16;
#pragma unroll
                for (int e = 0; e < 4; e++) kpre[u][e] = make_float4(0.f, 0.f, 0.f, 0.f);
                if (ks + 96 * u < n_old) {
#pragma unroll
                    for (int e = 0; e < 4; e++) kpre[u][e] = ldg4(kc + (ko + 4 * e));
                }
            };
            kload(0);
            {
                float a0 = 0.f, a1 = 0.f;
#pragma unroll
                for (int i = 0; i < 4; i++) {
                    const StepCtx cx = load_ctx(xs, binfo, 2 * (4 * cw + i), lane);
                    a0 = mstep(rq[i], cx, a0); a1 = mstep(rq[4 + i], cx, a1);
                }
                a0 = g01_sum(a0, lane); a1 = g01_sum(a1, lane);
                if (lane < 16) part[lane * NCONS + cw] = a0;
                if (lane < 8) part[(16 + lane) * NCONS + cw] = a1;
            }
            cs.cbarrier();
            if (it == 0) { wait_ge(&c->gw_flag, (unsigned)NCONS, c, p.err, ERR_STAGE); xloc = (p.flags & 128) != 0 && lds_ld(&c->xcd_ok) != 0; }
            if (cw == 0) {
                const int r = min(lane, 23);
                float a = 0.f;
#pragma unroll
                for (int w = 0; w < NCONS; w++) a += part[r * NCONS + w];
                a *= cs.rstd_staged(ssl);
                const float rc = c->rope_c[r], rs = c->rope_s[r];
                const float o = dppf<0xB1>(a);
                const float y = (lane & 1) ? fmaf(o, rs, a * rc) : fmaf(-o, rs, a * rc);
                if (lane < 24) {
                    const int n = lane < 16 ? 128 * h + 16 * s + lane : lane < 20 ? EQD + 128 * g + 4 * j + (lane - 16) : EQD + EKD + 128 * g + 4 * j + (lane - 20);
                    publish_b(p.G, (EQD + 2 * EKD) * 8u, (unsigned)n, tag, y, xloc);
                    if (lane >= 16) (lane < 20 ? kc : vc)[(size_t)pos * EHD + (n & 127)] = y;
                }
            }
            cs.published(tl, tlev ? 28 : -1);
            if (T) tl(1);
            kload(1);
            float2 vpre[16];
#pragma unroll
            for (int u = 0; u < 16; u++) {
                vpre[u] = make_float2(0.f, 0.f);
                if (cw + 12 * u < n_old) {
                    const fv2 v = *(const __attribute__((address_space(1))) fv2*)(vc + ((unsigned)(j_lo + cw + 12 * u) * EHD + lane * 2));
                    vpre[u] = make_float2(v.x, v.y);
                }
            }
            wait_ge(&c->qkv_flag, (unsigned)l + 1u, c, p.err, ERR_STAGE);
            if (T) tl(2);
            {
                float qv[16];
#pragma unroll
                for (int e = 0; e < 4; e++) { const float4 v = *reinterpret_cast<const float4*>(qkvn + part_ * 16 + 4 * e); qv[4 * e] = v.x; qv[4 * e + 1] = v.y; qv[4 * e + 2] = v.z; qv[4 * e + 3] = v.w; }
                auto dot16 = [&](const float4 (&kk)[4]) {
                    float sacc = 0.f;
#pragma unroll
                    for (int e = 0; e < 4; e++) { sacc = fmaf(qv[4 * e], kk[e].x, sacc); sacc = fmaf(qv[4 * e + 1], kk[e].y, sacc); sacc = fmaf(qv[4 * e + 2], kk[e].z, sacc); sacc = fmaf(qv[4 * e + 3], kk[e].w, sacc); }
                    return group8_sum_e(sacc);
                };
#pragma unroll
                for (int u = 0; u < NKP; u++) {
                    const float sv = dot16(kpre[u]);
                    const int i = ks + 96 * u;
                    if (part_ == 0 && i < n_old) sc[i] = sv * scale;
                }
                for (int i0 = 96 * NKP; i0 < n_old; i0 += 96 * NKP) {
#pragma unroll
                    for (int u = 0; u < NKP; u++) {
                        const int i = i0 + ks + 96 * u;
                        const unsigned ko = (unsigned)(j_lo + min(i, last_old)) * EHD + part_ * 16;
#pragma unroll
                        for (int e = 0; e < 4; e++) kpre[u][e] = make_float4(0.f, 0.f, 0.f, 0.f);
                        if (i < n_old) {
#pragma unroll
                            for (int e = 0; e < 4; e++) kpre[u][e] = ldg4(kc + (ko + 4 * e));
                        }
                    }
#pragma unroll
                    for (int u = 0; u < NKP; u++) {
                        const float sv = dot16(kpre[u]);
                        const int i = i0 + ks + 96 * u;
                        if (part_ == 0 && i < n_old) sc[i] = sv * scale;
                    }
                }
                if (cw == 0) {
                    float4 kk[4];
#pragma unroll
                    for (int e = 0; e < 4; e++) kk[e] = *reinterpret_cast<const float4*>(qkvn + 128 + part_ * 16 + 4 * e);
                    const float sv = dot16(kk);
                    if (t12 == 0) sc[n_old] = sv * scale;
                }
            }
            if (T) tl(26);
            cs.cbarrier();
            if (T) tl(27);
            {
                const int n = n_old + 1;
                float mx = -INFINITY;
                for (int i = lane; i < n; i += 64) mx = fmaxf(mx, sc[i]);
                mx = wave_max_e(mx);
                float2 o = make_float2(0.f, 0.f); float lsum = 0.f;
                const int iu = cw + 12 * (lane & 15);
                const float pv = iu < n_old ? expf(sc[iu] - mx) : 0.f;
#pragma unroll
                for (int u = 0; u < 16; u++) {
                    const float pr_ = rlf(pv, u); const float2 vv = vpre[u];
                    o.x = fmaf(pr_, vv.x, o.x); o.y = fmaf(pr_, vv.y, o.y); lsum += pr_;
                }
                for (int b0 = 192; b0 < n_old; b0 += 192) {
#pragma unroll
                    for (int u = 0; u < 16; u++) {
                        vpre[u] = make_float2(0.f, 0.f);
                        if (b0 + cw + 12 * u < n_old) {
                            const fv2 v = *(const __attribute__((address_space(1))) fv2*)(vc + ((unsigned)(j_lo + b0 + cw + 12 * u) * EHD + lane * 2));
                            vpre[u] = make_float2(v.x, v.y);
                        }
                    }
                    const int ib = b0 + cw + 12 * (lane & 15);
                    const float pb = ib < n_old ? expf(sc[ib] - mx) : 0.f;
#pragma unroll
                    for (int u = 0; u < 16; u++) {
                        const float pr_ = rlf(pb, u); const float2 vv = vpre[u];
                        o.x = fmaf(pr_, vv.x, o.x); o.y = fmaf(pr_, vv.y, o.y); lsum += pr_;
                    }
                }
                if (cw == 0) {
                    const float pr_ = expf(sc[n_old] - mx); const float2 vv = *reinterpret_cast<const float2*>(qkvn + 256 + lane * 2);
                    o.x = fmaf(pr_, vv.x, o.x); o.y = fmaf(pr_, vv.y, o.y); lsum += pr_;
                }
                po[cw * 64 + lane] = o;
                if (lane == 0) pl[cw] = lsum;
            }
            if (T) tl(23);
            cs.cbarrier();
            if (T) tl(25);
            if (lane < 32) {
                const float4* po4 = reinterpret_cast<const float4*>(po);
                float4 so = make_float4(0.f, 0.f, 0.f, 0.f); float sl = 0.f;
#pragma unroll
                for (int q = 0; q < 12; q++) { const float4 a = po4[q * 32 + lane]; so.x += a.x; so.y += a.y; so.z += a.z; so.w += a.w; sl += pl[q]; }
                const float inv = 1.0f / sl;
                const float v[4] = {so.x * inv, so.y * inv, so.z * inv, so.w * inv};
                to_digits(v, lane, xs + (8 * cw + (lane >> 3)) * 128, binfo + 8 * cw + (lane >> 3));
            }
            if (T) tl(3);
            {
                StepCtx cx[2];
#pragma unroll
                for (int i = 0; i < 2; i++) cx[i] = load_ctx(xs, binfo, 8 * cw + 2 * i, lane);
#pragma unroll
                for (int i = 0; i < WO_PK; i++) {
                    int sl_; const unsigned char* bb = cs.slot_wait(cs.P + i, 2 * REC, sl_);
                    float a = mstep(bb, false, lane, cx[0], 0.f); a = mstep(bb + REC, false, lane, cx[1], a);
                    cs.slot_release(sl_);
                    a = g01_sum(a, lane);
                    if (lane < 16) publish_b(p.PW, NPW * ED * 8u, (unsigned)(h * ED + 384 * s + 16 * (2 * cw + i) + lane), tag, a, false);
                }
                cs.P += WO_PK;
                cs.published(tl, tlev ? 29 : -1);
            }
            if (T) tl(4);
            continue;
        }
        if (op == EOP_W13) {
            constexpr int NPRE = 3;
            RecR rw[4 * NPRE];
#pragma unroll
            for (int ti = 0; ti < NPRE; ti++) {
                int s0, s1;
                const unsigned char* b0 = cs.slot_wait(cs.P + 2 * ti, 2 * REC, s0);
                rw[4 * ti] = rec_read(b0, false, lane); rw[4 * ti + 1] = rec_read(b0 + REC, false, lane);
                cs.slot_release(s0);
                const unsigned char* b1 = cs.slot_wait(cs.P + 2 * ti + 1, 2 * REC, s1);
                rw[4 * ti + 2] = rec_read(b1, false, lane); rw[4 * ti + 3] = rec_read(b1 + REC, false, lane);
                cs.slot_release(s1);
            }
            cs.all_gather<true>(p.H1, p.SS1, tag, 2u * (unsigned)l + 1u, xs, ssl, binfo, tl, T);
            if (T) tl(5);
            StepCtx cx[4];
#pragma unroll
            for (int i = 0; i < 4; i++) cx[i] = load_ctx(xs, binfo, 2 * (4 * cw + i), lane);
            if (T) tl(24);
#pragma unroll
            for (int ti = 0; ti < NPRE; ti++) {
                float a = 0.f;
#pragma unroll
                for (int i = 0; i < 4; i++) a = mstep(rw[4 * ti + i], cx[i], a);
                a = g01_sum(a, lane);
                if (lane < 16) part[(16 * ti + lane) * NCONS + cw] = a;
            }
#pragma unroll 1
            for (int ti = NPRE; ti < 4; ti++) {
                int s0, s1;
                const unsigned char* b0 = cs.slot_wait(cs.P + 2 * ti, 2 * REC, s0);
                const unsigned char* b1 = cs.slot_wait(cs.P + 2 * ti + 1, 2 * REC, s1);
                float a = mstep(b0, false, lane, cx[0], 0.f); a = mstep(b0 + REC, false, lane, cx[1], a);
                a = mstep(b1, false, lane, cx[2], a); a = mstep(b1 + REC, false, lane, cx[3], a);
                cs.slot_release(s0); cs.slot_release(s1);
                a = g01_sum(a, lane);
                if (lane < 16) part[(16 * ti + lane) * NCONS + cw] = a;
            }
            {
                int s2; const unsigned char* b2 = cs.slot_wait(cs.P + 8, 4 * REC_H, s2);
                float a = 0.f;
#pragma unroll
                for (int i = 0; i < 4; i++) a = mstep(b2 + i * REC_H, true, lane, cx[i], a);
                cs.slot_release(s2);
                a = g01_sum(a, lane);
                if (lane < 8) part[(64 + lane) * NCONS + cw] = a;
            }
            cs.P += W13_PK;
            cs.cbarrier();
            if (cw < 2) {
                const int r = min(64 * cw + lane, 71);
                float a = 0.f;
#pragma unroll
                for (int w = 0; w < NCONS; w++) a += part[r * NCONS + w];
                a *= cs.rstd_staged(ssl);
                const float up = dppf<0xB1>(a);
                if ((lane & 1) == 0 && 64 * cw + lane < 72) publish_b(p.A, EF * 8u, (unsigned)(1152 * g + 36 * j + (r >> 1)), tag, silu_e(a) * up, xloc);
            }
            cs.published(tl, tlev ? 30 : -1);
            if (T) tl(6);
            continue;
        }
        if (op == EOP_W2) {
            RecR r2[9];
#pragma unroll
            for (int i = 0; i < W2_PK; i++) {
                int sl_; const unsigned char* bb = cs.slot_wait(cs.P + i, 3 * REC, sl_);
#pragma unroll
                for (int k = 0; k < 3; k++) r2[3 * i + k] = rec_read(bb + k * REC, false, lane);
                cs.slot_release(sl_);
            }
            wait_ge(&c->xa_flag, (unsigned)l + 1u, c, p.err, ERR_STAGE);
            if (T) tl(7);
            const int ksl = cw % 6, tg = cw / 6;
            if (lane < 48) {
                const float4 v4 = *reinterpret_cast<const float4*>(xa + 32 * (6 * ksl + (lane >> 3)) + 4 * (lane & 7));
                const float v[4] = {v4.x, v4.y, v4.z, v4.w};
                to_digits(v, lane, xs + (8 * cw + (lane >> 3)) * 128, binfo + 8 * cw + (lane >> 3));
            }
            StepCtx cx[3];
#pragma unroll
            for (int i = 0; i < 3; i++) cx[i] = load_ctx(xs, binfo, 8 * cw + 2 * i, lane);
#pragma unroll
            for (int i = 0; i < W2_PK; i++) {
                float a = mstep(r2[3 * i], cx[0], 0.f); a = mstep(r2[3 * i + 1], cx[1], a); a = mstep(r2[3 * i + 2], cx[2], a);
                a = g01_sum(a, lane);
                if (lane < 16) part2[(16 * (3 * tg + i) + lane) * 6 + ksl] = a;
            }
            cs.P += W2_PK;
            cs.cbarrier();
            if (cw < 2) {
                const int r = min(64 * cw + lane, 95);
                float a = 0.f;
#pragma unroll
                for (int w = 0; w < 6; w++) a += part2[r * 6 + w];
                if (64 * cw + lane < 96) publish_b(p.P2, NP2 * ED * 8u, (unsigned)(g * ED + 96 * j + r), tag, a, false);
            }
            cs.published(tl, tlev ? 31 : -1);
            if (T) tl(14);
            continue;
        }
        const float rstd = cs.all_gather<false>(p.H0, p.SS0, tag_base + (unsigned)p.n_layers, 2u * (unsigned)p.n_layers, xs, ssl, binfo, tl, false);
        XA xr; xr.load(reinterpret_cast<const float*>(xs), lane, 64 + (lane >> 1), lane & 1);
        const int n_pass = lm_packets(p.vocab);
        PassA Qa, Qb;
        cs.fetch(cs.P, Qa);
#pragma unroll 1
        for (int t = 0; t < n_pass; t++) {
            const int q = cw + NCONS * t;
            if (t + 1 < n_pass) cs.fetch(cs.P + t + 1, Qb);
            if (q < npass_lm) {
                const float r = wave_sum_e(Cons::dot(Qa, xr)) * rstd;
                const int n = row0_lm + q;
                if (p.logits_out && lane == 0) p.logits_out[n] = r;
                if (r > best || (r == best && n < best_i)) { best = r; best_i = n; }
            }
            Qa = Qb;
        }
        cs.P += (unsigned)n_pass;
    }
    if (lane0 == 0) { c->best_val[cw] = best; c->best_idx[cw] = best_i; }
    cs.cbarrier();
    if (cw == 0 && lane0 == 0) {
        float bv = c->best_val[0]; int bi = c->best_idx[0];
        for (int w = 1; w < NCONS; w++) { const float v = c->best_val[w]; const int ii = c->best_idx[w]; if (v > bv || (v == bv && ii < bi)) { bv = v; bi = ii; } }
        p.part_val[b] = bv; p.part_idx[b] = bi;
    }
    if (cw == 0) tl(15);
}

__global__ __launch_bounds__(NTHR, 1) void decode_engine_kernel(const EngParams p) {
    extern __shared__ __attribute__((aligned(16))) unsigned char lds[];
    EngCtl* c = reinterpret_cast<EngCtl*>(lds + L_CTL);
    const int tid = threadIdx.x, lane = tid & 63, wave = __builtin_amdgcn_readfirstlane(tid >> 6);
    if (tid < (int)(sizeof(EngCtl) / 4)) reinterpret_cast<unsigned*>(c)[tid] = 0u;
    for (int i = tid; i < p.n_layers * (int)(sizeof(EngLayerTab) / 8); i += NTHR) reinterpret_cast<u64*>(lds + L_TAB)[i] = reinterpret_cast<const u64*>(p.layers)[i];
    if (tid == 0) c->xcc_id = __builtin_amdgcn_s_getreg((20) | (0 << 6) | ((4 - 1) << 11));
    __syncthreads();
    Tl tl; tl.on = p.tl != nullptr && lane == 0; tl.buf = p.tl ? p.tl + (size_t)blockIdx.x * 32 : nullptr;
    if (wave == 0) {
        tl(19);
        eng_loader(p, c, (unsigned)(uintptr_t)(lds + L_RING), lane, tl);
    } else if (wave == 1) {
        eng_comm(p, c, lds, lane, tl);
        if (blockIdx.x == 0 && lane == 0) {
            const unsigned sv = *p.serial; asm volatile("" ::: "memory"); *p.serial = sv + 1u;
            if (p.flags & ENGF_ARGMAX_IN) { const int pv_ = *p.pos_rw; asm volatile("" ::: "memory"); *p.pos_rw = pv_ + 1; }
        }
    } else {
        eng_consumer(p, c, lds, wave - 2, lane, tl);
    }
}

__global__ __launch_bounds__(256) void eng_hidden_kernel(const u64* __restrict__ H, const u64* __restrict__ SS, float eps, float* __restrict__ out) {
    __shared__ float red[256];
    const int t = threadIdx.x;
    red[t] = __uint_as_float((unsigned)SS[t]);
    __syncthreads();
    for (int s = 128; s > 0; s >>= 1) { if (t < s) red[t] += red[t + s]; __syncthreads(); }
    const float rstd = 1.0f / sqrtf(red[0] / (float)ED + eps);
    const int k = blockIdx.x * 256 + t;
    out[k] = __uint_as_float((unsigned)H[k]) * (1.0f / 512.0f) * rstd;
}

}

hipError_t launch_eng_hidden(const EngParams& p, float* out, hipStream_t s) {
    const bool even = ((2 * p.n_layers) & 1) == 0;
    eng_hidden_kernel<<<dim3(ED / 256), dim3(256), 0, s>>>(even ? p.H0 : p.H1, even ? p.SS0 : p.SS1, p.eps, out);
    return hipGetLastError();
}

bool eng_geometry_ok(int D, int n_heads, int n_kv, int hd, int ffn, int vocab, int max_seq) {
    return D == ED && n_heads == ENH && n_kv == ENKV && hd == EHD && ffn == EF && vocab > 0 && vocab % NCU == 0 && max_seq > 0 && max_seq <= SC_MAX;
}
size_t eng_stream_bytes(int n_layers, int vocab) { return cu_stream_bytes(n_layers, vocab) * NCU; }
int eng_lds_bytes() { return L_TOTAL; }

static constexpr size_t ST_H0 = 0, ST_H1 = ST_H0 + (size_t)ED * 8, ST_G = ST_H1 + (size_t)ED * 8, ST_PW = ST_G + (size_t)(EQD + 2 * EKD) * 8,
                        ST_A = ST_PW + (size_t)NPW * ED * 8, ST_P2 = ST_A + (size_t)EF * 8, ST_SS0 = ST_P2 + (size_t)NP2 * ED * 8, ST_SS1 = ST_SS0 + (size_t)NCU * 8, ST_XC = ST_SS1 + (size_t)NCU * 8, ST_SERIAL = ST_XC + (size_t)NCU * 8, ST_ERR = ST_SERIAL + 256, ST_TOTAL = ST_ERR + 256;
size_t eng_state_bytes() { return ST_TOTAL; }
void eng_state_carve(unsigned char* st, EngParams* p) {
    p->H0 = reinterpret_cast<unsigned long long*>(st + ST_H0); p->H1 = reinterpret_cast<unsigned long long*>(st + ST_H1);
    p->XC = reinterpret_cast<unsigned long long*>(st + ST_XC);
    p->SS0 = reinterpret_cast<unsigned long long*>(st + ST_SS0); p->SS1 = reinterpret_cast<unsigned long long*>(st + ST_SS1);
    p->G = reinterpret_cast<unsigned long long*>(st + ST_G); p->PW = reinterpret_cast<unsigned long long*>(st + ST_PW);
    p->A = reinterpret_cast<unsigned long long*>(st + ST_A); p->P2 = reinterpret_cast<unsigned long long*>(st + ST_P2);
    p->serial = reinterpret_cast<unsigned*>(st + ST_SERIAL); p->err = reinterpret_cast<unsigned*>(st + ST_ERR);
}

hipError_t launch_eng_pack(const Q4W& w, int op, int layer, int n_layers, unsigned char* stream, int vocab, hipStream_t s) {
    if (w.fmt != WFMT_Q4_0 || !w.qs || !w.sc) return hipErrorInvalidValue;
    int off_bytes, N, K;
    switch (op) {
    case EOP_QKV: off_bytes = OFF_QKV; N = EQD + 2 * EKD; K = ED; break;
    case EOP_WO: off_bytes = OFF_WO; N = ED; K = EQD; break;
    case EOP_W13: off_bytes = OFF_W13; N = 2 * EF; K = ED; break;
    case EOP_W2: off_bytes = OFF_W2; N = ED; K = EF; break;
    case EOP_LM: off_bytes = 0; N = vocab; K = ED; break;
    case EOP_WOB: off_bytes = 0; N = ED; K = EQD; break;
    default: return hipErrorInvalidValue;
    }
    if (w.N != N || w.K != K) return hipErrorInvalidValue;
    if (op == EOP_LM) eng_pack_lm_kernel<<<dim3(lm_passes(vocab), NCU), dim3(64), 0, s>>>(w, stream, (size_t)n_layers * LAYER_BYTES, vocab);
    else if (op == EOP_WOB) eng_pack_kernel<<<dim3(op_packets(op) * NCONS * 4, NCU), dim3(64), 0, s>>>(w, op, stream, (size_t)layer * WOB_LAYER_BYTES);
    else eng_pack_kernel<<<dim3(op_packets(op) * NCONS * 4, NCU), dim3(64), 0, s>>>(w, op, stream, (size_t)layer * LAYER_BYTES + off_bytes);
    return hipGetLastError();
}

hipError_t eng_occupancy(int* blocks_per_cu) {
    hipError_t e = hipFuncSetAttribute(reinterpret_cast<const void*>(decode_engine_kernel), hipFuncAttributeMaxDynamicSharedMemorySize, 160 * 1024);
    if (e != hipSuccess) return e;
    return hipOccupancyMaxActiveBlocksPerMultiprocessor(blocks_per_cu, reinterpret_cast<const void*>(decode_engine_kernel), NTHR, L_TOTAL);
}

hipError_t launch_decode_engine(const EngParams& p, hipStream_t s) {
    static DevOnce attr_done;
    const int dev = vox_current_device();
    if (!attr_done.done(dev)) {
        hipError_t e = hipFuncSetAttribute(reinterpret_cast<const void*>(decode_engine_kernel), hipFuncAttributeMaxDynamicSharedMemorySize, 160 * 1024);
        if (e != hipSuccess) return e;
        attr_done.set(dev);
    }
    decode_engine_kernel<<<dim3(NCU), dim3(NTHR), L_TOTAL, s>>>(p);
    attn_form_note(ATTN_FORM_ENGINE);
    return hipGetLastError();
}

}
```

voxtral-mini-realtime-rs_amd/csrc/vox_kernels.h:

```cpp
#pragma once
#include <hip/hip_runtime.h>
#include <atomic>
struct DevOnce {
    std::atomic<uint64_t> mask{0};
    bool done(int dev) const { return (mask.load(std::memory_order_acquire) >> (dev & 63)) & 1ull; }
    void set(int dev) { mask.fetch_or(1ull << (dev & 63), std::memory_order_release); }
};
static inline int vox_current_device() { int d = 0; if (hipGetDevice(&d) != hipSuccess) { (void)hipGetLastError(); d = 0; } return d; }
#include <stdint.h>

namespace vox {

struct Q4W {
    const uint4* qs;
    const uint16_t* sc;
    int N, K, nb;
    int fmt;
    const uint4* qt = nullptr; const uint16_t* st = nullptr;
};
enum WFmt { WFMT_Q4_0 = 0, WFMT_BF16 = 1, WFMT_BF16X2 = 2, WFMT_F32 = 3 };

enum Epi { EPI_STORE = 0, EPI_RESID = 1, EPI_SWIGLU = 2, EPI_ROPE_KV = 3, EPI_ARGMAX = 4, EPI_GELU = 5, EPI_SWIGLU_XF = 6, EPI_RESID_XF = 7,
           EPI_ROPE_ROWS = 8,
           EPI_ROPE_KV_PAGED = 9,
           EPI_ROPE_KV_RING = 10,
           EPI_ROPE_KV_PAGED_BF16 = 12, EPI_ROPE_KV_PAGED_RING_BF16 = 13,
           EPI_ROPE_KV_PAGED_RING = 11 };
enum Pro { PRO_NONE = 0, PRO_RMS = 1, PRO_RMS_MUL = 2,
           PRO_RMS_MUL_SUM = 3 };

struct GemvParams {
    Q4W w;
    const float* x; int x_stride;
    float* out; int out_stride;
    const float* bias;
    const float* resid; int resid_stride;
    const float* gamma; const float* mul; float eps;
    long long* zero_acc; int zero_n;
    const long long* xacc; float* x_out;
    const int* pos_ptr; int pos_off;
    const float* rope_cos; const float* rope_sin; int hd;
    int n_q, n_k;
    float* kcache; float* vcache; int cache_head_stride;
    float* part_val; int* part_idx;
    int tl_slot;
    int rope_mask;
};
hipError_t launch_q4_gemv(const GemvParams& p, int n_rows_x, int pro, int epi, int R, hipStream_t s);
const char* q4_gemv_kernel_name(int K, int pro, int epi, int R);
int q4_gemv_default_R(int N, int K, int epi);
int q4_gemv_grid(int N, int R);
int q4_gemv_nwv(int K, int epi);
int q4_gemv_grid_k(int N, int K, int R, int epi);
int dense_gemv_grid(int N);

struct GemmParams {
    Q4W w;
    const float* x; int x_stride; int M;
    float* out; int out_stride;
    const float* bias;
    const float* resid; int resid_stride;
    const uint4* xf;
    uint16_t* xf_scratch; size_t xf_scratch_bytes;
    const float* ssq_part; int n_part; float norm_eps;
    uint16_t* xf_out; const float* xf_w; const float* xf_w2; float* ssq_out;
    const int* pos; const float* rope_cos; const float* rope_sin; int hd, n_q, n_kv; float* kc; float* vc; long kv_seq_stride; int kv_head_stride;
    const int* kv_row;
    const int* kv_pos;
    const int* rope_member; int rope_mask;
    int tl_slot;
    int ksplit;
    float* kz_scratch; size_t kz_scratch_bytes;
    int rope_seq_rows;
    int wide_mt; long xf_gstride , xf_out_gstride , ssq_part_gstride, ssq_out_gstride ;
    int wide_rows;
    int kv_bf16;
};
struct WidePlan { int kz, sps, ntw; };
bool q4_wide_plan(const Q4W& w, int mt, int epi, WidePlan* pl);
size_t q4_wide_planes_bytes(const Q4W& w, int mt, const WidePlan& pl);
hipError_t launch_q4_wide(const GemmParams& p, int epi, hipStream_t s);
hipError_t launch_q4_tile_build(Q4W w, uint4* qt, uint16_t* st, hipStream_t s);
hipError_t launch_q4_gemm(const GemmParams& p, int epi, hipStream_t s, bool* fused_rope = nullptr);
hipError_t launch_dense2_gemm(const GemmParams& p, int epi, hipStream_t s);
hipError_t launch_transpose(const float* in, int R, int C, float* out, hipStream_t s);
int q4_skinny_resid_xf_parts(int N);

hipError_t launch_q4_repack(const uint8_t* raw, uint4* qs, uint16_t* sc, int64_t n_blocks, int nb, int row_mul, int row_add, hipStream_t s);
hipError_t launch_q4_dequant(Q4W w, float* out, hipStream_t s);
hipError_t launch_rms_norm(const float* x, int x_stride, int rows, int dim, const float* gamma, const float* mul,
                           float eps, float* out, int out_stride, hipStream_t s);
hipError_t launch_rms_norm_sumk(float* x, int x_stride, int rows, int dim, const float* part, size_t part_stride, int ksplit, const float* gamma, float eps, float* out, int out_stride, hipStream_t s);
int q4_skinny_mt2_plan(const Q4W& w, int M);
hipError_t launch_xf_rows(const float* x, int x_stride, int M, int K, uint16_t* xf, hipStream_t s);
hipError_t launch_q4_skinny_mt2_planes(const GemmParams& p, int KZ, hipStream_t s);
hipError_t launch_splitk_finish_resid(const float* planes, int KZ, int M, int N, float* x, int x_stride, hipStream_t s);
hipError_t launch_splitk_finish_swiglu_xf(const float* planes, int KZ, int M, int N, const float* bias, uint16_t* xf, hipStream_t s);
hipError_t launch_splitk_finish_rope_kv(const float* planes, int KZ, int M, int N, float* q_out, int q_stride, int n_q, int n_kv, int hd, int pos_off,
                                        const float* cos_t, const float* sin_t, float* kc, float* vc, int head_stride, hipStream_t s);
hipError_t launch_rms_norm_xf_sumk(float* x, int x_stride, int rows, int dim, const float* planes, int kz, const float* gamma, const float* mul, float eps, uint16_t* xf, hipStream_t s);
hipError_t launch_rms_norm_xf(const float* x, int x_stride, int rows, int dim, const float* gamma, const float* mul,
                              float eps, uint16_t* xf, hipStream_t s);
hipError_t launch_rope(float* buf, int M, int stride, int n_rot, int hd, int pos_off, const float* cos_t,
                       const float* sin_t, hipStream_t s, int seq_rows = 0, const int* row_pos = nullptr);
hipError_t launch_kv_store(const float* buf, int M, int stride, int k_col, int n_kv, int hd, int pos_off,
                           float* kcache, float* vcache, int cache_head_stride, hipStream_t s, int seq_rows = 0, long kv_seq_stride = 0);

struct AttnParams {
    const float* q; int q_stride;
    const float* k; const float* v;
    int kv_row_stride, kv_head_stride;
    float* out; int out_stride;
    int M, kv_len, n_heads, n_kv_heads, offset, window;
    const int* pos_ptr;
    int pos_per_seq; int q_seq_stride, out_seq_stride; long kv_seq_stride;
    const int* kv_row;
    const int* seq_len;
    const int* seq_row_off;
    uint16_t* out_xf_tiles; long out_xf_tile_stride;
    uint16_t* out_xf;
    long out_xf_gstride;
    int prefer_gqa;
    int no_xcd_remap;
    int tl_slot;
    int spec_zero;
    int spec_rows;
    const float* prefix_k; const float* prefix_v; int prefix_len, prefix_row_stride, prefix_head_stride;
    const int* page_tab; int page_tab_stride, page_shift, score_rows; long page_floats;
    int page_tab_len;
    int kv_bf16;
};
hipError_t launch_attn_prefill(const AttnParams& p, int hd, hipStream_t s, int n_seq = 1);
bool attn_prefill_prefix_ok(const AttnParams& p, int hd, int n_seq);
bool attn_prefill_small_ok(const AttnParams& p, int hd, int n_seq);
hipError_t launch_attn_decode(const AttnParams& p, int hd, int max_seq, hipStream_t s, int n_seq = 1);
bool attn_decode_takes_gqa(int hd, int n_heads, int n_kv_heads);
hipError_t attn_decode_gqa_max_seq(int* out);
hipError_t launch_attn_decode_paged(const AttnParams& p, int hd, hipStream_t s, int n_seq);
hipError_t launch_attn_decode_ring(const AttnParams& p, int hd, int cap, hipStream_t s, int n_seq = 1);
bool attn_wo_supported(const AttnParams& p, const Q4W& wo, int hd, int max_seq);
hipError_t launch_attn_wo(const AttnParams& p, const Q4W& wo, long long* acc, int max_seq, hipStream_t s);
enum AttnForm { ATTN_FORM_PREFILL_SMALL, ATTN_FORM_PREFILL_MFMA, ATTN_FORM_PREFILL_F32, ATTN_FORM_DECODE, ATTN_FORM_DECODE_SPEC, ATTN_FORM_DECODE_GQA, ATTN_FORM_WO,
                ATTN_FORM_ENGINE, ATTN_FORM_STREAM_RING, ATTN_FORM_GROUP_RESAMPLE, ATTN_FORM_STREAM_RESAMPLE,
                ATTN_FORM_DECODE_PAGED, ATTN_FORM_DECODE_GQA_PAGED,
                ATTN_FORM_DECODE_RING,
                ATTN_FORM_DECODE_PAGED_RING, ATTN_FORM_DECODE_GQA_PAGED_RING,
                ATTN_FORM_DECODE_PAGED_BF16, ATTN_FORM_DECODE_GQA_PAGED_BF16,
                ATTN_FORM_DECODE_PAGED_RING_BF16, ATTN_FORM_DECODE_GQA_PAGED_RING_BF16,
                ATTN_FORM_COUNT };
void attn_form_note(AttnForm f);
void attn_form_counts(unsigned long long out[ATTN_FORM_COUNT]);
enum GemmForm { GEMM_FORM_GEMV_R1, GEMM_FORM_GEMV_R2, GEMM_FORM_GEMV_R4, GEMM_FORM_DENSE_GEMV, GEMM_FORM_SKINNY, GEMM_FORM_SKINNY_MT, GEMM_FORM_SKINNY_MT2, GEMM_FORM_XF_ROWS,
                GEMM_FORM_SPLITK_FINISH, GEMM_FORM_TILE_11, GEMM_FORM_TILE_12, GEMM_FORM_TILE_21, GEMM_FORM_TILE_22, GEMM_FORM_TILE_21_TB, GEMM_FORM_TILE_22_TB, GEMM_FORM_K32,
                GEMM_FORM_BIG, GEMM_FORM_BIG_ROPE, GEMM_FORM_DENSE2, GEMM_FORM_WIDE, GEMM_FORM_COUNT };
void gemm_form_counts(unsigned long long out[GEMM_FORM_COUNT]);

hipError_t launch_conv1d_gelu(const float* in, int Cin, int L, const float* w, const float* b, int Cout, float* out,
                              int out_token_major, hipStream_t s);

struct MelTables { const float* window; const float* cos_t; const float* sin_t; const float* fb; const int* fb_lo; const int* fb_hi; };
hipError_t launch_mel(const float* audio, long n, long left, long right, const float* scale_ptr, MelTables t,
                      float* out, int T, int transposed, hipStream_t s);
hipError_t launch_resample_matrix(const double* H, int new_len, int fft_in, int fft_out, float* At, hipStream_t s);
hipError_t launch_resample(const float* x, long n_in, const float* At, int fft_in, int fft_out, int delay, float* out, long n_out, hipStream_t s);
hipError_t launch_absmax(const float* x, long n, float target_peak, float* scale_out, hipStream_t s);
hipError_t launch_absmax_group(const float* x, long n, unsigned* group_max_cell, hipStream_t s);
hipError_t launch_group_scale(const unsigned* group_max, const int* unit_group, int n, float target, float* unit_scale, hipStream_t s);

hipError_t launch_embed(Q4W tok, const int* ids, int n, const float* audio, int D, const int* pos_ptr, int id_off,
                        int a_off, float* out, hipStream_t s);
hipError_t launch_argmax_final(const float* part_val, const int* part_idx, int n_parts, int* tokens, int* pos_ptr,
                               int tok_off, int inc, hipStream_t s);
hipError_t launch_argmax_embed(const float* part_val, const int* part_idx, int n_parts, int* tokens, int* pos_ptr, Q4W tok,
                               const float* audio, int D, float* h, hipStream_t s);
hipError_t launch_rope_kv_batch(float* qkv, int n, int stride, int n_q, int n_kv, int hd, const int* pos, const float* cos_t, const float* sin_t,
                                float* kcache, float* vcache, long seq_stride, int head_stride, hipStream_t s);
hipError_t launch_argmax_embed_batch(const float* logits, int n, int vocab, int* tokens, int tok_stride, int* pos, const int* seq_len, Q4W tok,
                                     const float* audio, long audio_seq_stride, int D, float* h, hipStream_t s,
                                     uint16_t* xf = nullptr, const float* xf_w = nullptr, float* ssq_out = nullptr,
                                     long xf_group_stride = 0, int ssq_group_stride = 0,
                                     const long* audio_off = nullptr);
struct SlotStepParams {
    const float* logits; int vocab;
    int* tokens; int tok_stride; const int* clip_len;
    int* slot_clip; int* slot_qpos; const int* queue; int q_stride;
    int* pos; int* kv_row; int n_clips; int first_pos;
    Q4W tok; const float* audio; const long* audio_off; int D;
    const float* h0;
    float* h;
    uint16_t* xf; const float* xf_w; float* ssq_out; long xf_group_stride; int ssq_group_stride;
    int init;
};
hipError_t launch_argmax_embed_slots(const SlotStepParams& p, int n_slots, hipStream_t s);
struct BatchTapParams {
    const float* logits; int vocab;
    const int* slot_clip; int clip0; const int* pos; const int* seq_len;
    const int* clip_unit; int n_clips;
    float* out; int* rows; int n_units, max_rows, first_pos;
};
hipError_t launch_batch_tap(const BatchTapParams& p, int n_rows, hipStream_t s);
hipError_t launch_occupy(int workgroups, int micros, hipStream_t s);
hipError_t launch_add_rows(const float* a, const float* b, float* out, long n, hipStream_t s);
hipError_t launch_gelu(float* x, long n, hipStream_t s);
hipError_t launch_argmax_rows(const float* x, int rows, int V, int* out, hipStream_t s);

struct EngLayerTab { const float* attn_norm; const float* ffn_norm; const float* ada_mul; float* kc; float* vc; };
struct EngParams {
    const unsigned char* stream; size_t cu_stride;
    const EngLayerTab* layers; int n_layers;
    const float* h_in;
    const float* final_norm;
    const int* pos_ptr; int pos_off;
    const float* rope_cos; const float* rope_sin;
    int max_seq, window; float eps;
    unsigned long long *H0, *H1, *G, *PW, *A, *P2;
    unsigned long long *SS0, *SS1;
    unsigned long long* XC;
    unsigned* serial; unsigned* err;
    float* part_val; int* part_idx;
    int* tokens; int* pos_rw; const uint4* tok_qs; const uint16_t* tok_sc; int tok_nb; const float* audio;
    float* logits_out;
    int vocab;
    unsigned long long* tl; int tl_layer;
    int flags;
    int ag_delay_ticks;
    int pace_ticks;
};
bool eng_geometry_ok(int D, int n_heads, int n_kv, int hd, int ffn, int vocab, int max_seq);
size_t eng_stream_bytes(int n_layers, int vocab);
size_t eng_state_bytes();
hipError_t launch_eng_pack(const Q4W& w, int op, int layer, int n_layers, unsigned char* stream, int vocab, hipStream_t s);
void eng_state_carve(unsigned char* state, EngParams* p);
hipError_t launch_decode_engine(const EngParams& p, hipStream_t s);
hipError_t launch_eng_hidden(const EngParams& p, float* out, hipStream_t s);
hipError_t eng_occupancy(int* blocks_per_cu);
int eng_lds_bytes();

struct EngBParams {
    const unsigned char* stream;
    const unsigned char* stream_wo;
    const EngLayerTab* layers; int n_layers;
    long kv_seq_stride;
    const float* h_in; int h_stride; int n_rows;
    const float* final_norm;
    const int* pos;
    const int* kv_row;
    const float* rope_cos; const float* rope_sin;
    int max_seq, window; float eps;
    unsigned char *XH0, *XH1;
    float *SS0, *SS1;
    unsigned long long* G;
    unsigned char* XO;
    float* PW;
    unsigned char* XA;
    float* P2;
    unsigned *F0, *F1, *FO, *FW, *FA, *F2;
    unsigned long long* XC; unsigned* serial; unsigned* err;
    uint16_t* xf_out; float* ssq_out;
    unsigned long long* tl; int tl_layer;
    int flags;
};
size_t engb_state_bytes();
size_t engb_wo_stream_bytes(int n_layers);
void engb_state_carve(unsigned char* state, EngBParams* p);
hipError_t engb_state_init(unsigned char* state, hipStream_t s);
hipError_t launch_decode_engine_b16(const EngBParams& p, hipStream_t s);
hipError_t launch_decode_engine_b16x2(const EngBParams& a, const EngBParams& b, hipStream_t s);
hipError_t engb_occupancy(int* blocks_per_cu);
hipError_t engb_prepare_kernels();
hipError_t launch_engb_ssq_fold(const float* ssq256, float* ssq16, hipStream_t s);
int engb_lds_bytes();
int engb_lds_bytes2();

void knobs_load_once();
void knobs_reload();
#define VOX_NO_PK_F32 __attribute__((target("no-packed-fp32-ops")))
const char* knob_str(const char* name);

hipError_t tl_configure(unsigned long long* buf, int n_slots, int n_waves);
int tl_slots_used();
void tl_slot_meta(int slot, int out[4]);

enum StreamWord { STRM_POS = 0,
                  STRM_ENC_POS = 1,
                  STRM_FRAME = 2,
                  STRM_HEAD = 3,
                  STRM_TICKS = 4,
                  STRM_TAP_ROWS = 5,
                  STRM_WORDS = 16 };
struct TokenScore { float logprob, margin; int runner_up, id; };
static const int VOX_ALTS_MAX = 8;
struct TokenAlt { int id; float logprob; };
struct TokenAlts { float entropy; int n; TokenAlt alt[VOX_ALTS_MAX]; };
struct StreamMember {
    const float* samples; float gain;
    int* state;
    float *kring, *vring;
    int* tokens;
    float* tap; int tap_max;
    struct TokenScore* scores; int scores_cap;
    struct TokenAlts* alts; int alts_cap, alts_k;
};
hipError_t launch_stream_mel(const StreamMember* mem, const int* order, int n, int ring_mask, long left, MelTables t, int halo_back, int n_frames, float* out, long slot_stride,
                             hipStream_t s);
hipError_t launch_stream_resample(const float* in_ring, int in_mask, long n_in, const float* At, int fft_in, int fft_out, int delay, float* out_ring, int out_mask, long i0, int count,
                                  hipStream_t s);
hipError_t launch_stream_s16(const short* src, int count, float* ring, int mask, long w0, hipStream_t s);
struct StreamIngest {
    const float* in_ring; int in_mask;
    long n_in;
    const float* At; int fft_in, fft_out, delay;
    float* out_ring;
    long i0; int count;
};
hipError_t launch_stream_group_resample(const StreamIngest* desc, const StreamIngest* host, int n, int out_mask, hipStream_t s);
struct StreamS16 { const short* src; int count; float* ring; int mask; long w0; };
hipError_t launch_stream_group_s16(const StreamS16* desc, const StreamS16* host, int n, hipStream_t s);
struct StreamAttnParams {
    const float* qkv; int qkv_stride;
    const StreamMember* mem; const int* order; int n;
    size_t ring_off; int cap;
    const float* cos_t; const float* sin_t;
    float* out; int out_stride;
    int M, n_heads, window;
    int rope_mask;
    int rope_stride;
};
hipError_t launch_stream_attn(const StreamAttnParams& p, int hd, hipStream_t s);
hipError_t launch_stream_ring_init(const float* kv, int layers, int rows, int n_heads, int hd, int cap, float* kring, float* vring, hipStream_t s);
hipError_t launch_stream_embed(Q4W tok, const int* tokens, const float* audio_row, float* audio_keep, int keep_rows, int D, const int* state, float* h, hipStream_t s);
hipError_t launch_stream_embed_kept(Q4W tok, const int* tokens, const float* audio_keep, int keep_rows, int D, const int* state, float* h, hipStream_t s);
hipError_t launch_stream_advance(const float* part_val, const int* part_idx, int n_parts, int* tokens, int* state, int enc_rows, int frames, int cap, hipStream_t s);
struct StreamPages { const int* tab; int tab_stride, shift; int* page_out; int* in_page_out; int tab_len; };
hipError_t launch_stream_group_embed(Q4W tok, const StreamMember* mem, const int* order, int n, const float* audio, int D, float* h, uint16_t* xf, const float* xf_w,
                                     float* ssq_out, int* pos, int* kv_row, hipStream_t s, const StreamPages* pages = nullptr);
hipError_t launch_stream_pages_seed(const float* src_k, const float* src_v, int layers, int kv_heads, int rows, int hd, const int* tab, int page_shift, size_t layer_stride,
                                    float* pool_k, float* pool_v, hipStream_t s, bool kv_bf16 = false);
hipError_t launch_stream_group_advance(const float* logits, int vocab, const StreamMember* mem, const int* order, int n, int enc_rows, int frames, int cap, hipStream_t s);
hipError_t launch_score_rows(const float* x, int rows, int V, const int* ids, TokenScore* out, hipStream_t s);
hipError_t launch_stream_score(const float* logits, int vocab, const StreamMember* mem, const int* order, int n, int first_pos, hipStream_t s);
hipError_t launch_alts_rows(const float* x, int rows, int V, int k, TokenAlts* out, hipStream_t s);
hipError_t launch_stream_alts(const float* logits, int vocab, const StreamMember* mem, const int* order, int n, int first_pos, hipStream_t s);
hipError_t launch_records_rows(const float* x, int rows, int V, int k, TokenScore* scores, TokenAlts* alts, hipStream_t s);
struct BatchRecordsParams {
    const float* logits; int vocab;
    const int* slot_clip; int clip0; const int* pos; const int* seq_len;
    const int* rec_off; int n_clips, n_records, first_pos;
    TokenScore* scores; TokenAlts* alts; int k;
};
hipError_t launch_batch_records(const BatchRecordsParams& p, int n_rows, hipStream_t s);
struct StreamKeepParams {
    const StreamMember* mem; const int* order; int n;
    int layers, n_heads, hd, cap, rows;
    float* keep; size_t slot_stride;
};
size_t stream_keep_floats(int layers, int n_heads, int hd, int rows);
hipError_t launch_stream_keep(const StreamKeepParams& p, int restore, hipStream_t s);
enum SnapLayout { SNAP_FLAT = 0, SNAP_RING = 1, SNAP_PAGED = 2, SNAP_PAGED_RING = 3 };
struct SnapshotKvParams {
    float *cache_k, *cache_v; float *blob_k, *blob_v;
    int layers, heads, hd, lo, hi;
    int plane0, n_planes;
    int layout;
    size_t layer_stride, head_stride;
    int cap;
    const int* tab; int shift, tab_len;
    size_t page_floats;
    int kv_bf16;
};
bool snapshot_kv_pages_ok(const int* tab, int layout, int shift, int tab_len, int lo, int hi, int pool_pages, int* bad_page);
hipError_t launch_snapshot_kv(const SnapshotKvParams& p, int restore, hipStream_t s);

}
```

Measured before the change: 1505.

## Run multiple decode steps inside one persistent engine kernel launch

The persistent decode engine kernel now loops over up to N decode steps per launch (32 by default). Argmax partials go through a new device-side PVI exchange buffer and a step flag instead of a separate argmax/embed launch or graph replay per token. Tags become monotonic per step so the loader, comm and consumer waves can keep going across steps without the per-launch teardown and sync cost. Template variants specialise a lean many-step path. This risks subtle cross-step synchronisation bugs and adds register pressure.

```diff
diff --git a/voxtral-mini-realtime-rs_amd/csrc/vox_api.cpp b/voxtral-mini-realtime-rs_amd/csrc/vox_api.cpp
--- a/voxtral-mini-realtime-rs_amd/csrc/vox_api.cpp
+++ b/voxtral-mini-realtime-rs_amd/csrc/vox_api.cpp
@@ -700,13 +700,14 @@
     return VOX_OK;
 }
 
+static void engine_argmax_first(vox_model* m, EngParams* ep) {
+    ep->flags |= 65536; ep->h_in = nullptr; ep->tokens = m->d_tokens; ep->pos_rw = m->d_pos; ep->tok_qs = m->tok.w.qs; ep->tok_sc = m->tok.w.sc; ep->tok_nb = m->tok.w.nb; ep->audio = m->d_audio;
+}
 static int32_t decode_step_enqueue(vox_model* m, float* logits_out, bool eng, StepLaunch how = StepLaunch::StepAndArgmax) {
     const vox_model_cfg& c = m->cfg; hipStream_t s = m->ctx->stream;
     if (eng) {
         EngParams ep = engine_params(m, m->eng_offline, m->cache, m->d_h, m->d_pos, 0, logits_out);
-        if (how == StepLaunch::EngineArgmaxFirst) {
-            ep.flags |= 65536; ep.h_in = nullptr; ep.tokens = m->d_tokens; ep.pos_rw = m->d_pos; ep.tok_qs = m->tok.w.qs; ep.tok_sc = m->tok.w.sc; ep.tok_nb = m->tok.w.nb; ep.audio = m->d_audio;
-        }
+        if (how == StepLaunch::EngineArgmaxFirst) engine_argmax_first(m, &ep);
         HIPCHK(launch_decode_engine(ep, s));
         if (how == StepLaunch::StepAndArgmax) HIPCHK(launch_argmax_embed(m->d_part_val, m->d_part_idx, 256, m->d_tokens, m->d_pos, m->tok.w, m->d_audio, c.dec_dim, m->d_h, s));
         return VOX_OK;
@@ -792,12 +793,19 @@
     }
     return replay_rest(m, eng, done, plan.steps);
 }
-static int32_t steps_chained(vox_model* m, const ClipPlan& plan) {
-    hipStream_t s = m->ctx->stream;
-    const DecodeGraphs& g = graphs_for(m, {m->cache, m->d_audio, decode_unroll(true), StepLaunch::EngineArgmaxFirst});
-    VOXCHK(decode_step_enqueue(m, nullptr, true, StepLaunch::EngineAlone));
-    if (!g.exec[0]) { HIPCHK(hipStreamSynchronize(s)); VOXCHK(graph_capture(m, 0, 1, true)); }
-    VOXCHK(replay_rest(m, true, 1, plan.steps));
+static const int ENGINE_STEPS_DEFAULT = 32;
+static int engine_steps_knob() { const char* e = knob_str("VOX_ENGINE_STEPS"); return e && atoi(e) >= 1 ? std::min(atoi(e), ENGINE_MAX_ROWS) : 0; }
+static int32_t steps_chained(vox_model* m, const ClipPlan& plan, float* d_logits_all) {
+    hipStream_t s = m->ctx->stream; const size_t V = (size_t)m->cfg.vocab;
+    const int N = engine_steps_knob() ? engine_steps_knob() : ENGINE_STEPS_DEFAULT;
+    VOXCHK(decode_step_enqueue(m, d_logits_all ? d_logits_all + V : nullptr, true, StepLaunch::EngineAlone));
+    for (int done = 1; done < plan.steps;) {
+        const int n = std::min(N, plan.steps - done);
+        EngParams ep = engine_params(m, m->eng_offline, m->cache, nullptr, m->d_pos, 0, d_logits_all ? d_logits_all + (size_t)(done + 1) * V : nullptr);
+        engine_argmax_first(m, &ep); ep.n_steps = n; ep.logits_stride = (long long)V;
+        HIPCHK(launch_decode_engine(ep, s));
+        done += n; m->timings.graph_replays += n;
+    }
     HIPCHK(launch_argmax_final(m->d_part_val, m->d_part_idx, 256, m->d_tokens, m->d_pos, 1, 1, s));
     return VOX_OK;
 }
@@ -806,9 +814,10 @@
     if (plan.steps <= 0) return VOX_OK;
     VOXCHK(wo_acc_clear(m, s));
     HIPCHK(launch_embed(m->tok.w, m->d_tokens, 1, m->d_audio, c.dec_dim, m->d_pos, 0, 0, m->d_h, s));
-    if (plan.want_logits) return steps_eager_logits(m, plan, eng, d_logits_all);
     const char* k = knob_str("VOX_ENGINE_ARGMAX_IN");
-    return eng && !(k && k[0] == '0') ? steps_chained(m, plan) : steps_replayed(m, plan, eng);
+    const bool chained = eng && !(k && k[0] == '0');
+    if (plan.want_logits) return chained && engine_steps_knob() ? steps_chained(m, plan, d_logits_all) : steps_eager_logits(m, plan, eng, d_logits_all);
+    return chained ? steps_chained(m, plan, nullptr) : steps_replayed(m, plan, eng);
 }
 
 struct ClipRecords { vox_token_score* scores; vox_token_alts* alts; int k; };
diff --git a/voxtral-mini-realtime-rs_amd/csrc/vox_engine.hip b/voxtral-mini-realtime-rs_amd/csrc/vox_engine.hip
--- a/voxtral-mini-realtime-rs_amd/csrc/vox_engine.hip
+++ b/voxtral-mini-realtime-rs_amd/csrc/vox_engine.hip
@@ -37,13 +37,13 @@
 
 struct EngCtl {
     unsigned ring_ready[8], ring_done[8];
-    unsigned xs0_flag, xs1_flag, xa_flag, qkv_flag;
+    unsigned step_flag, ag_flag_o, xa_flag, qkv_flag;
     unsigned cbar, dead, gathering, gw_flag;
     unsigned xcd_ok, xcc_id, ag_flag, pub_cnt;
-    float rstd0, rstd1, pad1, pad2;
+    float rstd0, rstd1; unsigned tl_tag, pad2;
     float best_val[16]; int best_idx[16];
     float h_own[16], h1_own[16];
-    unsigned ag_done, pad_q[3];
+    unsigned ag_done, tag0, tl_tag15, pad_q;
     float rope_c[24], rope_s[24];
 };
 constexpr int L_RING = 0;
@@ -67,6 +67,11 @@
 static_assert(L_TAB % 16 == 0 && sizeof(EngLayerTab) == 40, "layer table");
 static_assert(L_XS % 16 == 0 && L_XA % 16 == 0 && L_QKVN % 16 == 0 && L_PO % 16 == 0 && L_CTL % 16 == 0 && L_BLK % 8 == 0 && 72 * 12 * 4 <= SC_MAX * 4 && 1152 * 4 + 96 * 6 * 4 <= SC_MAX * 4 + 12 * 128 * 4, "aligned carve");
 
+constexpr int ENGF_ARGMAX_IN = 65536;
+typedef const __attribute__((address_space(4))) EngParams* kparams_t;
+__device__ __forceinline__ kparams_t eng_kernargs() { kparams_t k = (kparams_t)__builtin_amdgcn_kernarg_segment_ptr(); asm volatile("" : "+s"(k)); return k; }
+__device__ __forceinline__ int eng_n_steps(const EngParams& p) { return (p.flags & ENGF_ARGMAX_IN) && p.n_steps > 1 ? p.n_steps : 1; }
+
 __device__ __forceinline__ void eng_loader(const EngParams& p, EngCtl* c, unsigned ring_lds, int lane, const Tl& tl) {
     Loader<EngCtl, NSLOT> ld; ld.c = c; ld.err = p.err; ld.ring_lds = ring_lds; ld.voff = (unsigned)lane * 16u; ld.thin = (p.flags & 1) != 0; ld.pace = (u64)p.pace_ticks;
     const bool fake = (p.flags & 2) != 0;
@@ -76,6 +81,11 @@
     if (p.flags & 2048) ld.depth = 1;
     const u64 base = (u64)p.stream;
     const unsigned n_layer_pk = (unsigned)p.n_layers * PK_LAYER, n_pk = n_layer_pk + (unsigned)lm_packets(p.vocab);
+    const u64 pace0 = ld.pace, pause0 = ld.pause_ticks; const int depth0 = ld.depth, n_steps = eng_n_steps(p);
+#pragma unroll 1
+    for (int t = 0; t < n_steps; t++) {
+    if (t > 0) { if (lds_ld(&c->dead)) break; ld.pace = pace0; ld.pause_ticks = pause0; ld.depth = depth0; }
+    const int tl_layer = t == p.tl_step ? p.tl_layer : -1;
     unsigned l = 0, r = 0;
     u64 off = 0;
 #pragma unroll 1
@@ -83,12 +93,13 @@
         int bytes = PK_A;
         if (pk < n_layer_pk) {
             if (r < PK_LAYER_M) bytes = PK_M;
-            if (r == 0 && (int)l == p.tl_layer) tl(16);
+            if (r == 0 && (int)l == tl_layer) tl(16);
         } else { ld.pace = 0; ld.pause_ticks = 0; ld.depth = 3; }
         const u64 src = fake ? base + (u64)blockIdx.x * PK_A : base + (u64)NCU * off + (u64)blockIdx.x * (u64)bytes;
         if (bytes == PK_M) ld.issue<PK_M>(src, lane, nodma); else ld.issue<PK_A>(src, lane, nodma);
         off += (u64)bytes;
-        if (++r == PK_LAYER) { if ((int)l == p.tl_layer) tl(17); r = 0; l++; }
+        if (++r == PK_LAYER) { if ((int)l == tl_layer) tl(17); r = 0; l++; }
+    }
     }
     ld.flush();
     tl(18);
@@ -118,13 +129,22 @@
     if (lane == 0) publish(ssq + b, tag, sq);
 }
 
-constexpr int ENGF_ARGMAX_IN = 65536;
-__device__ __forceinline__ float comm_next_input(const EngParams& p, int lane, unsigned own_k) {
+__device__ __forceinline__ float comm_next_input(const EngParams& p, EngCtl* ctl, int lane, unsigned own_k, int t, int cur, unsigned tag_prev) {
     float xv[4]; int xi[4];
-#pragma unroll
-    for (int u = 0; u < 4; u++) { xv[u] = as_g(p.part_val)[lane + 64 * u]; xi[u] = ((const __attribute__((address_space(1))) int*)(uintptr_t)p.part_idx)[lane + 64 * u]; }
-    const int cur = __builtin_amdgcn_readfirstlane(*p.pos_rw) + 1;
-    const float au = as_g(p.audio)[(size_t)cur * ED + own_k];
+    float au;
+    if (t == 0) {
+#pragma unroll
+        for (int u = 0; u < 4; u++) { xv[u] = as_g(p.part_val)[lane + 64 * u]; xi[u] = ((const __attribute__((address_space(1))) int*)(uintptr_t)p.part_idx)[lane + 64 * u]; }
+        au = as_g(p.audio)[(size_t)cur * ED + own_k];
+    } else {
+        au = as_g(p.audio)[(size_t)cur * ED + own_k];
+        float v[8];
+        lds_st(&ctl->gathering, 1u);
+        sweep<8>(p.PVI, 2u * NCU * 8u, tag_prev, [&](int u) { return lane + 64 * u; }, [&]() { return 0; }, false, v, ctl, p.err);
+        lds_st(&ctl->gathering, 0u);
+#pragma unroll
+        for (int u = 0; u < 4; u++) { xv[u] = v[u]; xi[u] = __float_as_int(v[4 + u]); }
+    }
     float bv = -INFINITY; int bi = 0x7fffffff;
 #pragma unroll
     for (int u = 0; u < 4; u++) if (xv[u] > bv || (xv[u] == bv && xi[u] < bi)) { bv = xv[u]; bi = xi[u]; }
@@ -149,34 +169,47 @@
     float* xa = reinterpret_cast<float*>(lds + L_XA); float* qkvn = reinterpret_cast<float*>(lds + L_QKVN);
     float* tmp = reinterpret_cast<float*>(lds + L_TMP);
     const EngLayerTab* tab = reinterpret_cast<const EngLayerTab*>(lds + L_TAB);
-    const unsigned tag_base = (*p.serial + 1u) * 64u;
+    unsigned tag_base = (*p.serial + 1u) * 64u;
     const bool PROBE_SMALL = (p.flags & 4) != 0;
-    const int own_r = min(lane0, OWN - 1);
-    const unsigned own_k = (unsigned)(OWN * b + own_r);
     const float* gwt = reinterpret_cast<const float*>(lds + L_GW);
+    int cur = (p.flags & ENGF_ARGMAX_IN) ? __builtin_amdgcn_readfirstlane(*p.pos_rw) + 1 : 0;
+    unsigned pub_t = 0, agd_t = 0;
+#pragma unroll 1
+    for (int steps_left = eng_n_steps(p), t = 0;; t = 1) {
     {
-        const float g0 = ld_gf(make_srd(p.n_layers > 0 ? tab[0].attn_norm : p.final_norm, ED * 4u), own_k) * (p.n_layers > 0 ? 1.0f : 512.0f);
-        const float hraw = (p.flags & ENGF_ARGMAX_IN) ? comm_next_input(p, lane0, own_k) : ld_gf(make_srd(p.h_in, ED * 4u), own_k);
-        comm_publish_rows(p, lane0, hraw, g0, p.H0, p.SS0, tag_base, c->h_own);
+        int lane_s = lane0; asm volatile("" : "+v"(lane_s));
+        const int own_r = min(lane_s, OWN - 1);
+        const unsigned own_k = (unsigned)(OWN * b + own_r);
+        float g0;
+        if (t == 0) g0 = ld_gf(make_srd(p.n_layers > 0 ? tab[0].attn_norm : p.final_norm, ED * 4u), own_k) * (p.n_layers > 0 ? 1.0f : 512.0f);
+        else {
+            if (lds_ld(&c->dead)) break;
+            wait_ge(&c->step_flag, tag_base, c, p.err, ERR_STAGE);
+            g0 = gwt[own_r];
+        }
+        const float hraw = (p.flags & ENGF_ARGMAX_IN) ? comm_next_input(p, c, lane_s, own_k, t, cur, tag_base - 64u + (unsigned)p.n_layers + 1u) : ld_gf(make_srd(p.h_in, ED * 4u), own_k);
+        comm_publish_rows(p, lane_s, hraw, g0, p.H0, p.SS0, tag_base, c->h_own);
     }
 #pragma unroll 1
     for (int st = 0; st <= 2 * p.n_layers; st++) {
         int lane = lane0; asm volatile("" : "+v"(lane));
-        const int l = st >> 1; const bool odd = st & 1, last = st == 2 * p.n_layers, T = l == p.tl_layer;
+        const int l = st >> 1; const bool odd = st & 1, last = st == 2 * p.n_layers;
         const unsigned tag = tag_base + (unsigned)l + 1u;
+        const bool T = p.tl != nullptr && tag == lds_ld(&c->tl_tag);
         if (odd) comm_probe_x(p, c, lane, p.H1, tag, tl, T);
         else comm_probe_x(p, c, lane, p.H0, tag - 1u, tl, false);
         lds_st(&c->gathering, 1u);
-        lds_st(&c->ag_flag, (unsigned)st + 1u);
+        lds_st(odd ? &c->ag_flag_o : &c->ag_flag, tag);
         if (T) tl(odd ? 11 : 8);
-        if (p.flags & (1 | 64)) wait_ge(&c->ag_done, NCONS * ((unsigned)st + 1u), c, p.err, ERR_STAGE);
+        agd_t += NCONS;
+        if (p.flags & (1 | 64)) wait_ge(&c->ag_done, agd_t, c, p.err, ERR_STAGE);
         lds_st(&c->gathering, 0u);
         if (last) break;
         if (!odd) {
             wait_ge(&c->gw_flag, (unsigned)NCONS, c, p.err, ERR_STAGE);
             const bool xloc_nt = (p.flags & 128) != 0 && (p.flags & 4096) != 0 && lds_ld(&c->xcd_ok) != 0;
             {
-                wait_ge(&c->pub_cnt, NCONS * (4u * (unsigned)l + 1u), c, p.err, ERR_STAGE);
+                pub_t += NCONS; wait_ge(&c->pub_cnt, pub_t, c, p.err, ERR_STAGE);
                 lds_st(&c->gathering, 1u);
                 float v[6];
                 sweep<6>(p.G, (EQD + 2 * EKD) * 8u, tag, [&](int u) { const int i = lane + 64 * u, seg = i >> 7, e = i & 127; return seg == 0 ? 128 * h + e : (seg == 1 ? EQD : EQD + EKD) + 128 * g + e; },
@@ -184,11 +217,11 @@
                 lds_st(&c->gathering, 0u);
 #pragma unroll
                 for (int u = 0; u < 6; u++) qkvn[lane + 64 * u] = v[u];
-                ENG_CFENCE(); lds_st(&c->qkv_flag, (unsigned)l + 1u);
+                ENG_CFENCE(); lds_st(&c->qkv_flag, tag);
             }
             if (T) tl(9);
             {
-                wait_ge(&c->pub_cnt, NCONS * (4u * (unsigned)l + 2u), c, p.err, ERR_STAGE);
+                pub_t += NCONS; wait_ge(&c->pub_cnt, pub_t, c, p.err, ERR_STAGE);
                 lds_st(&c->gathering, 1u);
                 float v[6];
                 sweep<6>(p.PW, NPW * ED * 8u, tag, [&](int u) { const int i = lane + 64 * u, hh = i / OWN, r = i - hh * OWN; return hh * ED + OWN * b + r; }, [&]() { return (lane & 31) * ED + OWN * b; }, PROBE_SMALL, v, c, p.err);
@@ -208,18 +241,18 @@
         } else {
             const bool xloc_nt = (p.flags & 128) != 0 && (p.flags & 4096) != 0 && lds_ld(&c->xcd_ok) != 0;
             {
-                wait_ge(&c->pub_cnt, NCONS * (4u * (unsigned)l + 3u), c, p.err, ERR_STAGE);
+                pub_t += NCONS; wait_ge(&c->pub_cnt, pub_t, c, p.err, ERR_STAGE);
                 lds_st(&c->gathering, 1u);
                 float v[18];
                 sweep<18>(p.A, EF * 8u, tag, [&](int u) { return 1152 * g + lane + 64 * u; }, [&]() { return 1152 * g + 36 * (lane & 31) + 35; }, PROBE_SMALL, v, c, p.err, xloc_nt);
 #pragma unroll
                 for (int u = 0; u < 18; u++) xa[lane + 64 * u] = v[u];
-                ENG_CFENCE(); lds_st(&c->xa_flag, (unsigned)l + 1u);
+                ENG_CFENCE(); lds_st(&c->xa_flag, tag);
                 lds_st(&c->gathering, 0u);
             }
             if (T) tl(12);
             {
-                wait_ge(&c->pub_cnt, NCONS * (4u * (unsigned)l + 4u), c, p.err, ERR_STAGE);
+                pub_t += NCONS; wait_ge(&c->pub_cnt, pub_t, c, p.err, ERR_STAGE);
                 lds_st(&c->gathering, 1u);
                 float v[2];
                 sweep<2>(p.P2, NP2 * ED * 8u, tag, [&](int u) { const int i = min(lane + 64 * u, NP2 * OWN - 1), pp = i / OWN, r = i - pp * OWN; return pp * ED + OWN * b + r; }, [&]() { return min(lane, NP2 - 1) * ED + OWN * b; }, PROBE_SMALL, v, c, p.err);
@@ -236,6 +269,20 @@
             if (T) tl(13);
         }
     }
+    tag_base += 64u; cur++;
+    if (--steps_left <= 0) break;
+    }
+}
+
+__device__ __forceinline__ const void* uni_ptr(const void* q) {
+    const u64 v = (u64)(uintptr_t)q;
+    return (const void*)(uintptr_t)(((u64)(unsigned)__builtin_amdgcn_readfirstlane((int)(unsigned)(v >> 32)) << 32) | (u64)(unsigned)__builtin_amdgcn_readfirstlane((int)(unsigned)v));
+}
+__device__ __forceinline__ float4 ld_c4(srd_t sd, unsigned k, bool sc1) { const fv4 v = sc1 ? __builtin_bit_cast(fv4, __builtin_amdgcn_raw_buffer_load_b128(sd, (int)(k * 4u), 0, 16)) : __builtin_bit_cast(fv4, __builtin_amdgcn_raw_buffer_load_b128(sd, (int)(k * 4u), 0, 0)); return make_float4(v.x, v.y, v.z, v.w); }
+__device__ __forceinline__ float2 ld_c2(srd_t sd, unsigned k, bool sc1) { const fv2 v = sc1 ? __builtin_bit_cast(fv2, __builtin_amdgcn_raw_buffer_load_b64(sd, (int)(k * 4u), 0, 16)) : __builtin_bit_cast(fv2, __builtin_amdgcn_raw_buffer_load_b64(sd, (int)(k * 4u), 0, 0)); return make_float2(v.x, v.y); }
+__device__ __forceinline__ void st_c1(srd_t sd, unsigned k, float y, bool local) {
+    if (local) __builtin_amdgcn_raw_buffer_store_b32(__float_as_uint(y), sd, (int)(k * 4u), 0, 0);
+    else __builtin_amdgcn_raw_buffer_store_b32(__float_as_uint(y), sd, (int)(k * 4u), 0, 16);
 }
 
 __device__ __forceinline__ f2 cvt2(unsigned w, bool hi) { return hi ? __builtin_amdgcn_cvt_pk_f32_fp8((int)w, true) : __builtin_amdgcn_cvt_pk_f32_fp8((int)w, false); }
@@ -386,8 +433,8 @@
     static __device__ __forceinline__ float dot(const PassA& P_, const XA& xr) { return fmaf(P_.s1, half_dot(P_.q1, xr.xh, xr.m8h), P_.s0 * block_dot(P_.q0, xr.x, xr.m8)); }
 
     template <bool DIGITS>
-    __device__ __forceinline__ float all_gather(const u64* src, const u64* ssq, unsigned tag, unsigned stage, unsigned char* xs, float* ssl, float2* binfo, const Tl& tl, bool T) {
-        wait_ge(&c->ag_flag, stage + 1u, c, p.err, ERR_STAGE);
+    __device__ __forceinline__ float all_gather(const u64* src, const u64* ssq, unsigned tag, unsigned* flag, unsigned flag_tag, unsigned char* xs, float* ssl, float2* binfo, const Tl& tl, bool T) {
+        wait_ge(flag, flag_tag, c, p.err, ERR_STAGE);
         const srd_t sd = make_srd(src, ED * 8u), qd = make_srd(ssq, NCU * 8u);
         int ln = lane; asm volatile("" : "+v"(ln));
         if (DIGITS) {
@@ -444,15 +491,11 @@
     float* part2 = reinterpret_cast<float*>(lds + L_XA + 1152 * 4);
     const float* qkvn = reinterpret_cast<const float*>(lds + L_QKVN);
     float* sc = reinterpret_cast<float*>(lds + L_SC); float2* po = reinterpret_cast<float2*>(lds + L_PO); float* pl = reinterpret_cast<float*>(lds + L_PL);
-    const unsigned tag_base = (*p.serial + 1u) * 64u;
-    const int pos = *p.pos_ptr + p.pos_off + ((p.flags & ENGF_ARGMAX_IN) ? 1 : 0);
-    const int j_lo = p.window >= 0 ? max(0, pos - p.window) : 0, n_old = pos - j_lo, last_old = max(n_old - 1, 0);
+    unsigned tag_base = (*p.serial + 1u) * 64u;
+    const unsigned tag_base0 = tag_base;
+    int pos = *p.pos_ptr + p.pos_off + ((p.flags & ENGF_ARGMAX_IN) ? 1 : 0);
     const int half = EHD / 2;
-    if (cw == 0 && lane0 < 24) {
-        float rc = 1.0f, rs = 0.0f;
-        if (lane0 < 20) { const int pr = lane0 < 16 ? 8 * s + (lane0 >> 1) : 2 * j + ((lane0 - 16) >> 1); rc = p.rope_cos[(size_t)pos * half + pr]; rs = p.rope_sin[(size_t)pos * half + pr]; }
-        c->rope_c[lane0] = rc; c->rope_s[lane0] = rs;
-    }
+    const bool many = eng_n_steps(p) > 1;
     const float scale = 1.0f / sqrtf((float)EHD);
     const int n_items = 3 * p.n_layers, npass_lm = lm_passes(p.vocab), row0_lm = lm_rows_per_cu(p.vocab) * b;
     {
@@ -460,7 +503,7 @@
         float* gwt = reinterpret_cast<float*>(lds + L_GW);
         const bool xchg = cw == NCONS - 1 && (p.flags & 128) != 0;
         const unsigned my = c->xcc_id;
-        if (xchg && lane0 == 0) publish(p.XC + b, tag_base, __uint_as_float(my));
+        if (xchg && lane0 == 0) publish(p.XC + b, tag_base0, __uint_as_float(my));
         const int l = cw + NCONS * (lane0 >> 4), r = lane0 & 15, lc = min(l, max(p.n_layers - 1, 0));
         const bool lok = r < OWN && l <= p.n_layers && (lane0 >> 4) < 3, lay = l < p.n_layers;
         const unsigned k = (unsigned)(OWN * b + min(r, OWN - 1));
@@ -475,7 +518,7 @@
             unsigned ok = 0;
             if (xchg) {
                 float v[1];
-                const bool got = sweep<1>(p.XC, NCU * 8u, tag_base, [&](int) { return 8 * (lane0 & 31) + g; }, [&]() { return 0; }, false, v, c, p.err);
+                const bool got = sweep<1>(p.XC, NCU * 8u, tag_base0, [&](int) { return 8 * (lane0 & 31) + g; }, [&]() { return 0; }, false, v, c, p.err);
                 ok = got && __all(__float_as_uint(v[0]) == my) ? 1u : 0u;
                 if (!ok && lane0 == 0) __hip_atomic_store(p.err + 1, 9u | ((unsigned)b << 8) | (my << 16), RLX, AG);
             }
@@ -484,19 +527,30 @@
         ENG_CFENCE();
         if (lane0 == 0) __hip_atomic_fetch_add(&c->gw_flag, 1u, RLX, WG);
     }
+    bool xloc = false;
+
+#pragma unroll 1
+    for (int steps_left = eng_n_steps(p);;) {
+    const kparams_t kp = eng_kernargs();
+    const int win = kp->window;
+    const int j_lo = win >= 0 ? max(0, pos - win) : 0, n_old = pos - j_lo, last_old = max(n_old - 1, 0);
+    int lane_s = lane0; asm volatile("" : "+v"(lane_s));
+    if (cw == 0 && lane_s < 24) {
+        float rc = 1.0f, rs = 0.0f;
+        if (lane_s < 20) { const int pr = lane_s < 16 ? 8 * s + (lane_s >> 1) : 2 * j + ((lane_s - 16) >> 1); rc = as_g(kp->rope_cos)[(size_t)pos * half + pr]; rs = as_g(kp->rope_sin)[(size_t)pos * half + pr]; }
+        c->rope_c[lane_s] = rc; c->rope_s[lane_s] = rs;
+    }
     float best = -INFINITY; int best_i = 0x7fffffff;
-    bool xloc = false;
-
 #pragma unroll 1
     for (int it = 0; it <= n_items; it++) {
         int lane = lane0; asm volatile("" : "+v"(lane));
         const int l = it / 3, op = it == n_items ? (int)EOP_LM : (it - 3 * l == 0 ? (int)EOP_QKV : it - 3 * l == 1 ? (int)EOP_W13 : (int)EOP_W2);
-        const bool T = l == p.tl_layer && cw == 0 && op != EOP_LM;
-        const int tlev = l == p.tl_layer ? 1 : 0;
         const unsigned tag = tag_base + (unsigned)l + 1u;
+        const int tlev = p.tl != nullptr && tag == lds_ld(&c->tl_tag) ? 1 : 0;
+        const bool T = tlev && cw == 0 && op != EOP_LM;
         const EngLayerTab* L = reinterpret_cast<const EngLayerTab*>(lds + L_TAB) + (op == EOP_LM ? 0 : l);
         if (op == EOP_QKV) {
-            const gf_p kc = as_g(L->kc) + (size_t)g * p.max_seq * EHD, vc = as_g(L->vc) + (size_t)g * p.max_seq * EHD;
+            const srd_t kd = make_srd(uni_ptr(L->kc + (size_t)g * p.max_seq * EHD), (unsigned)p.max_seq * EHD * 4u), vd = make_srd(uni_ptr(L->vc + (size_t)g * p.max_seq * EHD), (unsigned)p.max_seq * EHD * 4u);
             const int t12 = cw * 64 + lane;
             const int part_ = t12 & 7, ks = t12 >> 3;
             RecR rq[8];
@@ -514,7 +568,7 @@
                 cs.slot_release(s2);
                 cs.P += QKV_PK;
             }
-            cs.all_gather<true>(p.H0, p.SS0, tag - 1u, 2u * (unsigned)l, xs, ssl, binfo, tl, false);
+            cs.all_gather<true>(p.H0, p.SS0, tag - 1u, &c->ag_flag, tag, xs, ssl, binfo, tl, false);
             if (T) tl(0);
             constexpr int NKP = 2;
             float4 kpre[NKP][4];
@@ -524,7 +578,7 @@
                 for (int e = 0; e < 4; e++) kpre[u][e] = make_float4(0.f, 0.f, 0.f, 0.f);
                 if (ks + 96 * u < n_old) {
 #pragma unroll
-                    for (int e = 0; e < 4; e++) kpre[u][e] = ldg4(kc + (ko + 4 * e));
+                    for (int e = 0; e < 4; e++) kpre[u][e] = ld_c4(kd, ko + 4 * e, many);
                 }
             };
             kload(0);
@@ -553,7 +607,7 @@
                 if (lane < 24) {
                     const int n = lane < 16 ? 128 * h + 16 * s + lane : lane < 20 ? EQD + 128 * g + 4 * j + (lane - 16) : EQD + EKD + 128 * g + 4 * j + (lane - 20);
                     publish_b(p.G, (EQD + 2 * EKD) * 8u, (unsigned)n, tag, y, xloc);
-                    if (lane >= 16) (lane < 20 ? kc : vc)[(size_t)pos * EHD + (n & 127)] = y;
+                    if (lane >= 16) { const unsigned ro = (unsigned)pos * EHD + (unsigned)(n & 127); if (lane < 20) st_c1(kd, ro, y, xloc); else st_c1(vd, ro, y, xloc); }
                 }
             }
             cs.published(tl, tlev ? 28 : -1);
@@ -564,11 +618,11 @@
             for (int u = 0; u < 16; u++) {
                 vpre[u] = make_float2(0.f, 0.f);
                 if (cw + 12 * u < n_old) {
-                    const fv2 v = *(const __attribute__((address_space(1))) fv2*)(vc + ((unsigned)(j_lo + cw + 12 * u) * EHD + lane * 2));
+                    const float2 v = ld_c2(vd, (unsigned)(j_lo + cw + 12 * u) * EHD + lane * 2, many);
                     vpre[u] = make_float2(v.x, v.y);
                 }
             }
-            wait_ge(&c->qkv_flag, (unsigned)l + 1u, c, p.err, ERR_STAGE);
+            wait_ge(&c->qkv_flag, tag, c, p.err, ERR_STAGE);
             if (T) tl(2);
             {
                 float qv[16];
@@ -595,7 +649,7 @@
                         for (int e = 0; e < 4; e++) kpre[u][e] = make_float4(0.f, 0.f, 0.f, 0.f);
                         if (i < n_old) {
 #pragma unroll
-                            for (int e = 0; e < 4; e++) kpre[u][e] = ldg4(kc + (ko + 4 * e));
+                            for (int e = 0; e < 4; e++) kpre[u][e] = ld_c4(kd, ko + 4 * e, many);
                         }
                     }
 #pragma unroll
@@ -634,7 +688,7 @@
                     for (int u = 0; u < 16; u++) {
                         vpre[u] = make_float2(0.f, 0.f);
                         if (b0 + cw + 12 * u < n_old) {
-                            const fv2 v = *(const __attribute__((address_space(1))) fv2*)(vc + ((unsigned)(j_lo + b0 + cw + 12 * u) * EHD + lane * 2));
+                            const float2 v = ld_c2(vd, (unsigned)(j_lo + b0 + cw + 12 * u) * EHD + lane * 2, many);
                             vpre[u] = make_float2(v.x, v.y);
                         }
                     }
@@ -697,7 +751,7 @@
                 rw[4 * ti + 2] = rec_read(b1, false, lane); rw[4 * ti + 3] = rec_read(b1 + REC, false, lane);
                 cs.slot_release(s1);
             }
-            cs.all_gather<true>(p.H1, p.SS1, tag, 2u * (unsigned)l + 1u, xs, ssl, binfo, tl, T);
+            cs.all_gather<true>(p.H1, p.SS1, tag, &c->ag_flag_o, tag, xs, ssl, binfo, tl, T);
             if (T) tl(5);
             StepCtx cx[4];
 #pragma unroll
@@ -755,7 +809,7 @@
                 for (int k = 0; k < 3; k++) r2[3 * i + k] = rec_read(bb + k * REC, false, lane);
                 cs.slot_release(sl_);
             }
-            wait_ge(&c->xa_flag, (unsigned)l + 1u, c, p.err, ERR_STAGE);
+            wait_ge(&c->xa_flag, tag, c, p.err, ERR_STAGE);
             if (T) tl(7);
             const int ksl = cw % 6, tg = cw / 6;
             if (lane < 48) {
@@ -785,7 +839,7 @@
             if (T) tl(14);
             continue;
         }
-        const float rstd = cs.all_gather<false>(p.H0, p.SS0, tag_base + (unsigned)p.n_layers, 2u * (unsigned)p.n_layers, xs, ssl, binfo, tl, false);
+        const float rstd = cs.all_gather<false>(p.H0, p.SS0, tag_base + (unsigned)p.n_layers, &c->ag_flag, tag_base + (unsigned)p.n_layers + 1u, xs, ssl, binfo, tl, false);
         XA xr; xr.load(reinterpret_cast<const float*>(xs), lane, 64 + (lane >> 1), lane & 1);
         const int n_pass = lm_packets(p.vocab);
         PassA Qa, Qb;
@@ -797,30 +851,52 @@
             if (q < npass_lm) {
                 const float r = wave_sum_e(Cons::dot(Qa, xr)) * rstd;
                 const int n = row0_lm + q;
-                if (p.logits_out && lane == 0) p.logits_out[n] = r;
+                if (p.logits_out && lane == 0) p.logits_out[(size_t)((tag_base - lds_ld(&c->tag0)) >> 6) * (size_t)p.logits_stride + n] = r;
                 if (r > best || (r == best && n < best_i)) { best = r; best_i = n; }
             }
             Qa = Qb;
         }
         cs.P += (unsigned)n_pass;
     }
-    if (lane0 == 0) { c->best_val[cw] = best; c->best_idx[cw] = best_i; }
+    asm volatile("" : "+v"(lane_s));
+    if (lane_s == 0) { c->best_val[cw] = best; c->best_idx[cw] = best_i; }
     cs.cbarrier();
-    if (cw == 0 && lane0 == 0) {
-        float bv = c->best_val[0]; int bi = c->best_idx[0];
-        for (int w = 1; w < NCONS; w++) { const float v = c->best_val[w]; const int ii = c->best_idx[w]; if (v > bv || (v == bv && ii < bi)) { bv = v; bi = ii; } }
-        p.part_val[b] = bv; p.part_idx[b] = bi;
-    }
-    if (cw == 0) tl(15);
-}
-
-__global__ __launch_bounds__(NTHR, 1) void decode_engine_kernel(const EngParams p) {
+    if (cw == 0) {
+        const bool more = steps_left > 1;
+        if (more) asm volatile("s_waitcnt vmcnt(0)" ::: "memory");
+        if (lane_s == 0) {
+            float bv = c->best_val[0]; int bi = c->best_idx[0];
+            for (int w = 1; w < NCONS; w++) { const float v = c->best_val[w]; const int ii = c->best_idx[w]; if (v > bv || (v == bv && ii < bi)) { bv = v; bi = ii; } }
+            const kparams_t ke = eng_kernargs();
+            if (more) { const unsigned tg = tag_base + (unsigned)ke->n_layers + 1u; u64* pvi = (u64*)ke->PVI; publish(pvi + b, tg, bv); publish(pvi + NCU + b, tg, __int_as_float(bi)); }
+            else { ke->part_val[b] = bv; ke->part_idx[b] = bi; }
+        }
+        if (more) { ENG_CFENCE(); lds_st(&c->step_flag, tag_base + 64u); }
+        if (p.tl != nullptr && tag_base == lds_ld(&c->tl_tag15)) tl(15);
+    }
+    tag_base += 64u; pos++;
+    if (--steps_left <= 0 || lds_ld(&c->dead)) break;
+    }
+}
+
+enum { ENG_ONE = 0, ENG_MANY = 1, ENG_MANY_X = 2 };
+constexpr int ENG_MANY_FLAGS = 1 | 128 | 512 | 16384 | ENGF_ARGMAX_IN;
+template <int MODE>
+__global__ __launch_bounds__(NTHR, 1) void decode_engine_kernel(const EngParams p_) {
+    EngParams p = p_;
+    if (MODE == ENG_ONE) p.n_steps = 1; else { p.n_steps = max(p.n_steps, 2); p.flags |= ENGF_ARGMAX_IN; }
+    if (MODE == ENG_MANY) { p.flags &= ENG_MANY_FLAGS; p.tl = nullptr; p.tl_layer = -1; }
     extern __shared__ __attribute__((aligned(16))) unsigned char lds[];
     EngCtl* c = reinterpret_cast<EngCtl*>(lds + L_CTL);
     const int tid = threadIdx.x, lane = tid & 63, wave = __builtin_amdgcn_readfirstlane(tid >> 6);
     if (tid < (int)(sizeof(EngCtl) / 4)) reinterpret_cast<unsigned*>(c)[tid] = 0u;
     for (int i = tid; i < p.n_layers * (int)(sizeof(EngLayerTab) / 8); i += NTHR) reinterpret_cast<u64*>(lds + L_TAB)[i] = reinterpret_cast<const u64*>(p.layers)[i];
-    if (tid == 0) c->xcc_id = __builtin_amdgcn_s_getreg((20) | (0 << 6) | ((4 - 1) << 11));
+    if (tid == 0) {
+        c->xcc_id = __builtin_amdgcn_s_getreg((20) | (0 << 6) | ((4 - 1) << 11));
+        c->tag0 = (*p.serial + 1u) * 64u;
+        if (p.tl) c->tl_tag15 = (*p.serial + 1u + (unsigned)max(p.tl_step - 1, 0)) * 64u;
+        if (p.tl && p.tl_layer >= 0) c->tl_tag = (*p.serial + 1u + (unsigned)p.tl_step) * 64u + (unsigned)p.tl_layer + 1u;
+    }
     __syncthreads();
     Tl tl; tl.on = p.tl != nullptr && lane == 0; tl.buf = p.tl ? p.tl + (size_t)blockIdx.x * 32 : nullptr;
     if (wave == 0) {
@@ -829,8 +905,9 @@
     } else if (wave == 1) {
         eng_comm(p, c, lds, lane, tl);
         if (blockIdx.x == 0 && lane == 0) {
-            const unsigned sv = *p.serial; asm volatile("" ::: "memory"); *p.serial = sv + 1u;
-            if (p.flags & ENGF_ARGMAX_IN) { const int pv_ = *p.pos_rw; asm volatile("" ::: "memory"); *p.pos_rw = pv_ + 1; }
+            const int n_steps = eng_n_steps(p);
+            const unsigned sv = *p.serial; asm volatile("" ::: "memory"); *p.serial = sv + (unsigned)n_steps;
+            if (p.flags & ENGF_ARGMAX_IN) { const int pv_ = *p.pos_rw; asm volatile("" ::: "memory"); *p.pos_rw = pv_ + n_steps; }
         }
     } else {
         eng_consumer(p, c, lds, wave - 2, lane, tl);
@@ -863,11 +940,11 @@
 int eng_lds_bytes() { return L_TOTAL; }
 
 static constexpr size_t ST_H0 = 0, ST_H1 = ST_H0 + (size_t)ED * 8, ST_G = ST_H1 + (size_t)ED * 8, ST_PW = ST_G + (size_t)(EQD + 2 * EKD) * 8,
-                        ST_A = ST_PW + (size_t)NPW * ED * 8, ST_P2 = ST_A + (size_t)EF * 8, ST_SS0 = ST_P2 + (size_t)NP2 * ED * 8, ST_SS1 = ST_SS0 + (size_t)NCU * 8, ST_XC = ST_SS1 + (size_t)NCU * 8, ST_SERIAL = ST_XC + (size_t)NCU * 8, ST_ERR = ST_SERIAL + 256, ST_TOTAL = ST_ERR + 256;
+                        ST_A = ST_PW + (size_t)NPW * ED * 8, ST_P2 = ST_A + (size_t)EF * 8, ST_SS0 = ST_P2 + (size_t)NP2 * ED * 8, ST_SS1 = ST_SS0 + (size_t)NCU * 8, ST_XC = ST_SS1 + (size_t)NCU * 8, ST_PVI = ST_XC + (size_t)NCU * 8, ST_SERIAL = ST_PVI + (size_t)2 * NCU * 8, ST_ERR = ST_SERIAL + 256, ST_TOTAL = ST_ERR + 256;
 size_t eng_state_bytes() { return ST_TOTAL; }
 void eng_state_carve(unsigned char* st, EngParams* p) {
     p->H0 = reinterpret_cast<unsigned long long*>(st + ST_H0); p->H1 = reinterpret_cast<unsigned long long*>(st + ST_H1);
-    p->XC = reinterpret_cast<unsigned long long*>(st + ST_XC);
+    p->XC = reinterpret_cast<unsigned long long*>(st + ST_XC); p->PVI = reinterpret_cast<unsigned long long*>(st + ST_PVI);
     p->SS0 = reinterpret_cast<unsigned long long*>(st + ST_SS0); p->SS1 = reinterpret_cast<unsigned long long*>(st + ST_SS1);
     p->G = reinterpret_cast<unsigned long long*>(st + ST_G); p->PW = reinterpret_cast<unsigned long long*>(st + ST_PW);
     p->A = reinterpret_cast<unsigned long long*>(st + ST_A); p->P2 = reinterpret_cast<unsigned long long*>(st + ST_P2);
@@ -893,21 +970,35 @@
     return hipGetLastError();
 }
 
+static const void* eng_kernel(int mode) {
+    return mode == ENG_ONE ? reinterpret_cast<const void*>(decode_engine_kernel<ENG_ONE>) : mode == ENG_MANY ? reinterpret_cast<const void*>(decode_engine_kernel<ENG_MANY>) : reinterpret_cast<const void*>(decode_engine_kernel<ENG_MANY_X>);
+}
+static hipError_t eng_set_attrs() {
+    hipError_t e = hipSuccess;
+    for (int i = 0; i < 3 && e == hipSuccess; i++) e = hipFuncSetAttribute(eng_kernel(i), hipFuncAttributeMaxDynamicSharedMemorySize, 160 * 1024);
+    return e;
+}
 hipError_t eng_occupancy(int* blocks_per_cu) {
-    hipError_t e = hipFuncSetAttribute(reinterpret_cast<const void*>(decode_engine_kernel), hipFuncAttributeMaxDynamicSharedMemorySize, 160 * 1024);
+    hipError_t e = eng_set_attrs();
     if (e != hipSuccess) return e;
-    return hipOccupancyMaxActiveBlocksPerMultiprocessor(blocks_per_cu, reinterpret_cast<const void*>(decode_engine_kernel), NTHR, L_TOTAL);
+    int occ[3] = {0, 0, 0};
+    for (int i = 0; i < 3 && e == hipSuccess; i++) e = hipOccupancyMaxActiveBlocksPerMultiprocessor(&occ[i], eng_kernel(i), NTHR, L_TOTAL);
+    *blocks_per_cu = std::min(occ[0], std::min(occ[1], occ[2]));
+    return e;
 }
 
 hipError_t launch_decode_engine(const EngParams& p, hipStream_t s) {
     static DevOnce attr_done;
     const int dev = vox_current_device();
     if (!attr_done.done(dev)) {
-        hipError_t e = hipFuncSetAttribute(reinterpret_cast<const void*>(decode_engine_kernel), hipFuncAttributeMaxDynamicSharedMemorySize, 160 * 1024);
+        hipError_t e = eng_set_attrs();
         if (e != hipSuccess) return e;
         attr_done.set(dev);
     }
-    decode_engine_kernel<<<dim3(NCU), dim3(NTHR), L_TOTAL, s>>>(p);
+    const bool many = (p.flags & ENGF_ARGMAX_IN) && p.n_steps > 1;
+    if (!many) decode_engine_kernel<ENG_ONE><<<dim3(NCU), dim3(NTHR), L_TOTAL, s>>>(p);
+    else if ((p.flags & ~ENG_MANY_FLAGS) == 0 && !p.tl) decode_engine_kernel<ENG_MANY><<<dim3(NCU), dim3(NTHR), L_TOTAL, s>>>(p);
+    else decode_engine_kernel<ENG_MANY_X><<<dim3(NCU), dim3(NTHR), L_TOTAL, s>>>(p);
     attn_form_note(ATTN_FORM_ENGINE);
     return hipGetLastError();
 }
diff --git a/voxtral-mini-realtime-rs_amd/csrc/vox_kernels.h b/voxtral-mini-realtime-rs_amd/csrc/vox_kernels.h
--- a/voxtral-mini-realtime-rs_amd/csrc/vox_kernels.h
+++ b/voxtral-mini-realtime-rs_amd/csrc/vox_kernels.h
@@ -216,12 +216,16 @@
     unsigned long long *H0, *H1, *G, *PW, *A, *P2;
     unsigned long long *SS0, *SS1;
     unsigned long long* XC;
+    unsigned long long* PVI;
     unsigned* serial; unsigned* err;
     float* part_val; int* part_idx;
     int* tokens; int* pos_rw; const uint4* tok_qs; const uint16_t* tok_sc; int tok_nb; const float* audio;
     float* logits_out;
+    long long logits_stride;
+    int n_steps;
     int vocab;
     unsigned long long* tl; int tl_layer;
+    int tl_step;
     int flags;
     int ag_delay_ticks;
     int pace_ticks;
```

Result: no change. 1519 (median of 6 runs) (+0.9%).
